# haan6/fm-for-online-recommendation

Measured on NVIDIA B200. Metric: train samples/sec (fwd+bwd+update), higher is better.
Workload: dtype f32

## Files before the change

fm_for_online_recommendation_b200/csrc/fm_backward.cu:

```cuda
#include "fmb_common.cuh"
#include <cstdlib>
#include <cstring>
#include <cuda.h>

namespace {

struct BwdParams {
    const int32_t* skeys;
    const int32_t* perm;
    int64_t N;
    const float* xv;
    float* table;
    int F, k, rowp, kp4;
    int cu;
    int ql_log;
    unsigned long long fmagic;
    int fshift;
    const float* S;
    const float* gs;
    int use_fm2;
    const float* gvec;
    float lr;
    int mode;
    int s_pitch;
    int gs_stride;
    int32_t key_limit;
    float* G;
    int64_t Npad;
    long long* dbg;
    float astep;
    union {
        fmb::FtrlState ftrl;
        fmb::AdagradState ada;
    };
    int min_run1;
    float* inbox[8];
    int shard_G, shard_me;
    int64_t shard_N;
    const int4* run_list;
    const uint32_t* run_segc;
    int run_nseg, run_cap;
    int pdl;
};

template <bool ADA>
__device__ __forceinline__ float row_update(const BwdParams& p, float old, float g, int32_t key, int c) {
    if (ADA) {
        float* sp = p.ada.sums + (size_t)key * p.rowp + c;
        float sv = *sp;
        const float o = fmb::adagrad_update(old, g, sv, p.lr, p.ada.eps);
        *sp = sv;
        return o;
    }
    return fmb::apply_update_a(old, g, p.lr, p.astep, p.mode);
}

template <bool ADA>
__global__ void __launch_bounds__(256) fm_bwd_entry_kernel(BwdParams p) {
    const int q = threadIdx.x & ((1 << p.ql_log) - 1);
    const int64_t i = (int64_t)blockIdx.x * (256 >> p.ql_log) + (threadIdx.x >> p.ql_log);
    if (i >= p.N || q >= p.cu) return;
    const int32_t key = __ldg(p.skeys + i);
    if (key >= p.key_limit) return;
    const int32_t kprev = i > 0 ? __ldg(p.skeys + i - 1) : -1;
    const int32_t knext = i + 1 < p.N ? __ldg(p.skeys + i + 1) : -1;
    const int32_t e = __ldg(p.perm + i);
    const int b = (int)(((unsigned long long)(unsigned)e * p.fmagic) >> p.fshift);
    const float x = p.xv ? __ldg(p.xv + e) : 1.0f;
    const float d = __ldg(p.gs + (size_t)b * p.gs_stride);
    float* rowptr = p.table + (size_t)key * p.rowp + q * 4;
    const float4 v4 = *reinterpret_cast<const float4*>(rowptr);
    float4 s4 = make_float4(0.f, 0.f, 0.f, 0.f), g4 = s4;
    if (q * 4 < p.kp4) {
        s4 = __ldg(reinterpret_cast<const float4*>(p.S + (size_t)b * p.s_pitch + q * 4));
        if (p.gvec) g4 = __ldg(reinterpret_cast<const float4*>(p.gvec + (size_t)b * p.s_pitch + q * 4));
    }
    const float v[4] = {v4.x, v4.y, v4.z, v4.w}, s[4] = {s4.x, s4.y, s4.z, s4.w}, g[4] = {g4.x, g4.y, g4.z, g4.w};
    const bool two = p.use_fm2 && p.gvec;
    float a[4], c[4];
#pragma unroll
    for (int t = 0; t < 4; ++t) {
        const int j = q * 4 + t;
        a[t] = 0.f; c[t] = 0.f;
        if (j < p.k) {
            const float ej = __fmul_rn(v[t], x);
            if (p.use_fm2) a[t] = __fmul_rn(__fsub_rn(__fmul_rn(d, s[t]), __fmul_rn(d, ej)), x);
            if (p.gvec) c[t] = __fmul_rn(__fsub_rn(__fmul_rn(g[t], s[t]), __fmul_rn(g[t], ej)), x);
        } else if (j == p.k) {
            a[t] = __fmul_rn(d, x);
        }
    }
    if (key != kprev && key != knext) {
        float o[4];
#pragma unroll
        for (int t = 0; t < 4; ++t) {
            const int j = q * 4 + t;
            if (j < p.k) {
                const float gr = two ? __fadd_rn(__fadd_rn(0.f, a[t]), __fadd_rn(0.f, c[t]))
                                     : __fadd_rn(0.f, p.gvec ? c[t] : a[t]);
                o[t] = row_update<ADA>(p, v[t], gr, key, j);
            } else if (j == p.k) {
                o[t] = row_update<ADA>(p, v[t], __fadd_rn(0.f, a[t]), key, j);
            } else {
                o[t] = v[t];
            }
        }
        *reinterpret_cast<float4*>(rowptr) = make_float4(o[0], o[1], o[2], o[3]);
    } else {
#pragma unroll
        for (int t = 0; t < 4; ++t) {
            const int j = q * 4 + t;
            if (j > p.k) continue;
            if (two) {
                p.G[(size_t)j * p.Npad + i] = a[t];
                if (j < p.k) p.G[(size_t)(p.k + 1 + j) * p.Npad + i] = c[t];
            } else {
                p.G[(size_t)j * p.Npad + i] = (p.gvec && j < p.k) ? c[t] : a[t];
            }
        }
    }
}

template <int CU, bool ADA>
__global__ void __launch_bounds__(256) fm_bwd_entry1_kernel(BwdParams p) {
    const int64_t i = (int64_t)blockIdx.x * 256 + threadIdx.x;
    if (i >= p.N) return;
    const int32_t key = __ldg(p.skeys + i);
    if (key >= p.key_limit) return;
    const int32_t kprev = i > 0 ? __ldg(p.skeys + i - 1) : -1;
    const int32_t knext = i + 1 < p.N ? __ldg(p.skeys + i + 1) : -1;
    const int32_t e = __ldg(p.perm + i);
    const int b = (int)(((unsigned long long)(unsigned)e * p.fmagic) >> p.fshift);
    const float x = p.xv ? __ldg(p.xv + e) : 1.0f;
    const float d = __ldg(p.gs + (size_t)b * p.gs_stride);
    float* rowptr = p.table + (size_t)key * p.rowp;
    float v[CU * 4], s[CU * 4], g[CU * 4];
#pragma unroll
    for (int q = 0; q < CU; ++q) {
        const float4 v4 = *reinterpret_cast<const float4*>(rowptr + q * 4);
        v[q * 4] = v4.x; v[q * 4 + 1] = v4.y; v[q * 4 + 2] = v4.z; v[q * 4 + 3] = v4.w;
        float4 s4 = make_float4(0.f, 0.f, 0.f, 0.f), g4 = s4;
        if (q * 4 < p.kp4) {
            s4 = __ldg(reinterpret_cast<const float4*>(p.S + (size_t)b * p.s_pitch + q * 4));
            if (p.gvec) g4 = __ldg(reinterpret_cast<const float4*>(p.gvec + (size_t)b * p.s_pitch + q * 4));
        }
        s[q * 4] = s4.x; s[q * 4 + 1] = s4.y; s[q * 4 + 2] = s4.z; s[q * 4 + 3] = s4.w;
        g[q * 4] = g4.x; g[q * 4 + 1] = g4.y; g[q * 4 + 2] = g4.z; g[q * 4 + 3] = g4.w;
    }
    const bool two = p.use_fm2 && p.gvec;
    const bool single = key != kprev && key != knext;
    float o[CU * 4], o2[CU * 4];
#pragma unroll
    for (int j = 0; j < CU * 4; ++j) {
        float a = 0.f, c = 0.f;
        if (j < p.k) {
            const float ej = __fmul_rn(v[j], x);
            if (p.use_fm2) a = __fmul_rn(__fsub_rn(__fmul_rn(d, s[j]), __fmul_rn(d, ej)), x);
            if (p.gvec) c = __fmul_rn(__fsub_rn(__fmul_rn(g[j], s[j]), __fmul_rn(g[j], ej)), x);
        } else if (j == p.k) {
            a = __fmul_rn(d, x);
        }
        if (single) {
            if (j < p.k) {
                const float gr = two ? __fadd_rn(__fadd_rn(0.f, a), __fadd_rn(0.f, c)) : __fadd_rn(0.f, p.gvec ? c : a);
                o[j] = row_update<ADA>(p, v[j], gr, key, j);
            } else if (j == p.k) {
                o[j] = row_update<ADA>(p, v[j], __fadd_rn(0.f, a), key, j);
            } else {
                o[j] = v[j];
            }
        } else {
            o[j] = two ? a : ((p.gvec && j < p.k) ? c : a);
            o2[j] = c;
        }
    }
    if (single) {
#pragma unroll
        for (int q = 0; q < CU; ++q)
            *reinterpret_cast<float4*>(rowptr + q * 4) = make_float4(o[q * 4], o[q * 4 + 1], o[q * 4 + 2], o[q * 4 + 3]);
    } else {
#pragma unroll
        for (int j = 0; j < CU * 4; ++j) {
            if (j > p.k) continue;
            p.G[(size_t)j * p.Npad + i] = o[j];
            if (two && j < p.k) p.G[(size_t)(p.k + 1 + j) * p.Npad + i] = o2[j];
        }
    }
}


__device__ __forceinline__ void mbar_init(uint64_t* bar, int count) {
    asm volatile("mbarrier.init.shared::cta.b64 [%0], %1;\n" ::"r"((unsigned)__cvta_generic_to_shared(bar)), "r"(count));
}
__device__ __forceinline__ void mbar_expect_tx(uint64_t* bar, unsigned bytes) {
    asm volatile("mbarrier.arrive.expect_tx.shared::cta.b64 _, [%0], %1;\n" ::"r"((unsigned)__cvta_generic_to_shared(bar)), "r"(bytes) : "memory");
}
__device__ __forceinline__ bool mbar_wait(uint64_t* bar, unsigned parity) {
    const unsigned a = (unsigned)__cvta_generic_to_shared(bar);
    for (int spin = 0; spin < (1 << 20); ++spin) {
        unsigned ok;
        asm volatile("{\n\t.reg .pred p;\n\tmbarrier.test_wait.parity.shared::cta.b64 p, [%1], %2;\n\tselp.u32 %0, 1, 0, p;\n\t}\n"
                     : "=r"(ok) : "r"(a), "r"(parity) : "memory");
        if (ok) return true;
    }
    return false;
}
__device__ __forceinline__ void tma_g2s_2d(void* smem_dst, const CUtensorMap* tmap, int x, int y, uint64_t* bar) {
    asm volatile(
        "cp.async.bulk.tensor.2d.shared::cluster.global.mbarrier::complete_tx::bytes [%0], [%1, {%2, %3}], [%4];\n" ::"r"(
            (unsigned)__cvta_generic_to_shared(smem_dst)),
        "l"(tmap), "r"(x), "r"(y), "r"((unsigned)__cvta_generic_to_shared(bar))
        : "memory");
}

template <bool LIST, int RING_SE, int RING_NS, bool LONGM, bool ADA>
__device__ __forceinline__ void runs_body(const CUtensorMap& gmap, const BwdParams& p, int warps_per_block, int warp_f, int accs_n,
                                          int ring_comps, unsigned bid, unsigned nblocks, int segb_off) {
    constexpr int RING_SEP = RING_SE + 4;
    extern __shared__ __align__(128) float smem[];
    const int lane = threadIdx.x & 31, wib = threadIdx.x >> 5;
    const int64_t P0 = ((int64_t)bid * warps_per_block + wib) * 32;
    if (!LIST && P0 >= p.N) return;
    const bool two = p.use_fm2 && p.gvec;
    const int kc = p.k + 1;
    const int nv = kc + (two ? p.k : 0);
    const int stage_f = (ring_comps * RING_SEP + 31) & ~31;
    float* ring = smem + (size_t)wib * warp_f;
    uint64_t* bars = reinterpret_cast<uint64_t*>(ring + RING_NS * stage_f);
    float* accs = reinterpret_cast<float*>(bars + RING_NS);

    int32_t k0 = -2, k1 = -2;
    unsigned todo = 0;
    uint32_t lr = 0, ln = 0, lstep = 0;
    uint32_t* seg_base = reinterpret_cast<uint32_t*>(smem + segb_off);
    if (LIST) {
        lr = bid * warps_per_block + wib;
        lstep = nblocks * warps_per_block;
        for (int g = threadIdx.x; g < p.run_nseg; g += blockDim.x) seg_base[g] = __ldg(p.run_segc + (LONGM ? p.run_nseg : 0) + g);
        __syncthreads();
        if (wib == 0) {
            uint32_t carry = 0;
            for (int b0 = 0; b0 < p.run_nseg; b0 += 32) {
                const uint32_t v = b0 + lane < p.run_nseg ? seg_base[b0 + lane] : 0u;
                uint32_t inc = v;
#pragma unroll
                for (int o = 1; o < 32; o <<= 1) { const uint32_t t = __shfl_up_sync(0xffffffffu, inc, o); if (lane >= o) inc += t; }
                if (b0 + lane < p.run_nseg) seg_base[b0 + lane] = carry + inc - v;
                carry += __shfl_sync(0xffffffffu, inc, 31);
            }
            if (lane == 0) seg_base[p.run_nseg] = carry;
        }
        __syncthreads();
        const uint32_t total = seg_base[p.run_nseg];
        ln = total;
        if (wib >= warps_per_block) return;
        if (p.pdl) asm volatile("griddepcontrol.wait;\n" ::: "memory");
    } else {
        const int64_t pos = P0 + lane;
        k0 = pos < p.N ? __ldg(p.skeys + pos) : -2;
        k1 = pos + 32 < p.N ? __ldg(p.skeys + pos + 32) : -2;
        int32_t prev = __shfl_up_sync(0xffffffffu, k0, 1);
        int32_t next = __shfl_down_sync(0xffffffffu, k0, 1);
        const int32_t k1_0 = __shfl_sync(0xffffffffu, k1, 0);
        if (lane == 0) prev = P0 > 0 ? __ldg(p.skeys + P0 - 1) : -1;
        if (lane == 31) next = k1_0;
        todo = __ballot_sync(0xffffffffu, pos < p.N && k0 >= 0 && k0 < p.key_limit && k0 != prev && (k0 == next || p.min_run1));
    }
    bool bars_ready = false;
    unsigned phase = 0;

    while (LIST ? lr < ln : todo != 0) {
        int64_t s;
        int32_t key;
        int n0;
        if (LIST) {
            int lo = 0, hi = p.run_nseg;
            while (hi - lo > 1) { const int mid = (lo + hi) >> 1; if (seg_base[mid] <= lr) lo = mid; else hi = mid; }
            const uint32_t idx = lr - seg_base[lo];
            const int4 e = __ldg(p.run_list + (size_t)lo * p.run_cap + (LONGM ? (uint32_t)p.run_cap - 1u - idx : idx));
            lr += lstep;
            s = e.x; key = e.y; n0 = e.z;
        } else {
            const int bit = __ffs(todo) - 1;
            todo &= todo - 1;
            s = P0 + bit;
            key = __shfl_sync(0xffffffffu, k0, bit);
            const int t = bit + lane;
            const int32_t ka = __shfl_sync(0xffffffffu, k0, t & 31);
            const int32_t kb = __shfl_sync(0xffffffffu, k1, t & 31);
            const unsigned mm = __ballot_sync(0xffffffffu, (t < 32 ? ka : kb) == key);
            n0 = (mm == 0xffffffffu) ? 32 : __ffs(~mm) - 1;
        }
        long long t_start = 0, t_direct = 0, t_ring = 0, c_wait = 0, c_cons = 0, c_issue = 0;
        if (p.dbg) t_start = clock64();
        int run_len = 0;
        int32_t probe = -2;
        const int64_t ring0 = LONGM ? s : s + 32;
        if (LONGM) n0 = 0;
        const bool ringed = LONGM || n0 == 32;
        if (ringed) { const int64_t q = ring0 + 32 * (int64_t)(lane + 1) - 1; probe = q < p.N ? __ldg(p.skeys + q) : -2; }
        if (ringed && !bars_ready) {
            if (lane == 0) {
                for (int st = 0; st < RING_NS; ++st) mbar_init(bars + st, 1);
                asm volatile("fence.mbarrier_init.release.cluster;\n" ::: "memory");
            }
            __syncwarp();
            bars_ready = true;
        }

        for (int v0 = 0; v0 < nv; v0 += 32) {
            const int vl = v0 + lane;
            const bool active = vl < nv;
            const bool isB = vl >= kc;
            const int comp = isB ? vl - kc : vl;
            const float* src = p.G + (size_t)(active ? vl : 0) * p.Npad;
            (void)isB; (void)comp;
            float pold = 0.f;
            if (v0 == 0 && lane < kc && !p.shard_G) pold = p.table[(size_t)key * p.rowp + lane];
            float acc = 0.f;
            {
                const float* sp = src + s;
                float tv[16], tw[16];
#pragma unroll
                for (int u = 0; u < 16; ++u) tv[u] = (active && u < n0) ? __ldg(sp + u) : 0.f;
#pragma unroll
                for (int u = 0; u < 16; ++u) tw[u] = (active && 16 + u < n0) ? __ldg(sp + 16 + u) : 0.f;
#pragma unroll
                for (int u = 0; u < 16; ++u)
                    if (u < n0) acc = __fadd_rn(acc, tv[u]);
#pragma unroll
                for (int u = 0; u < 16; ++u)
                    if (16 + u < n0) acc = __fadd_rn(acc, tw[u]);
            }
            if (p.dbg) t_direct = clock64();
            run_len = n0;
            if (ringed) {
                int64_t c0 = ring0;
                const int mis = (int)(c0 & 3);
                int32_t pr = probe;
                bool ok = true;
                while (ok) {
                    const unsigned pm = __ballot_sync(0xffffffffu, pr == key);
                    const int full = (pm == 0xffffffffu) ? 32 : __ffs(~pm) - 1;
                    int part = 0;
                    if (full < 32) {
                        const int64_t q = c0 + 32 * (int64_t)full + lane;
                        const unsigned m3 = __ballot_sync(0xffffffffu, q < p.N && __ldg(p.skeys + q) == key);
                        part = (m3 == 0xffffffffu) ? 32 : __ffs(~m3) - 1;
                    }
                    const int wlen = 32 * full + part;
                    const int T = (wlen + RING_SE - 1) / RING_SE;
                    auto issue = [&](int tstage) {
                        if (lane == 0) {
                            const int st = tstage & (RING_NS - 1);
                            mbar_expect_tx(bars + st, (unsigned)(ring_comps * RING_SEP * 4));
                            tma_g2s_2d(ring + (size_t)st * stage_f, &gmap, (int)(c0 - mis + RING_SE * (int64_t)tstage), v0, bars + st);
                        }
                    };
                    for (int ts = 0; ts < T && ts < RING_NS; ++ts) issue(ts);
                    int32_t pr_next = -2;
                    if (full == 32) { const int64_t q = c0 + 1024 + 32 * (int64_t)(lane + 1) - 1; pr_next = q < p.N ? __ldg(p.skeys + q) : -2; }
                    for (int ts = 0; ts < T; ++ts) {
                        const int st = ts & (RING_NS - 1);
                        long long w0 = 0;
                        if (p.dbg) w0 = clock64();
                        if (!mbar_wait(bars + st, (phase >> st) & 1u)) { ok = false; break; }
                        phase ^= 1u << st;
                        long long w1 = 0;
                        if (p.dbg) { w1 = clock64(); c_wait += w1 - w0; }
                        const int n = min(RING_SE, wlen - RING_SE * ts);
                        if (active) {
                            const float4* b4 = reinterpret_cast<const float4*>(ring + (size_t)st * stage_f + lane * RING_SEP);
                            if (n == RING_SE) {
                                {
                                    const float4 q = b4[0];
                                    if (mis == 0) acc = __fadd_rn(acc, q.x);
                                    if (mis <= 1) acc = __fadd_rn(acc, q.y);
                                    if (mis <= 2) acc = __fadd_rn(acc, q.z);
                                    acc = __fadd_rn(acc, q.w);
                                }
#pragma unroll
                                for (int c = 0; c < RING_SE / 64; ++c) {
                                    constexpr int last = RING_SE / 64 - 1;
                                    const int nq = c == last ? 15 : 16;
                                    float4 tv[16];
#pragma unroll
                                    for (int u = 0; u < 16; ++u) if (u < nq) tv[u] = b4[1 + 16 * c + u];
#pragma unroll
                                    for (int u = 0; u < 16; ++u)
                                        if (u < nq) {
                                            acc = __fadd_rn(acc, tv[u].x); acc = __fadd_rn(acc, tv[u].y);
                                            acc = __fadd_rn(acc, tv[u].z); acc = __fadd_rn(acc, tv[u].w);
                                        }
                                }
                                {
                                    const float4 q = b4[RING_SE / 4];
                                    if (mis >= 1) acc = __fadd_rn(acc, q.x);
                                    if (mis >= 2) acc = __fadd_rn(acc, q.y);
                                    if (mis >= 3) acc = __fadd_rn(acc, q.z);
                                }
                            } else {
                                const int end = mis + n;
                                int e = 0;
                                if (mis) {
                                    const float4 q = b4[0];
                                    if (mis <= 1 && 1 < end) acc = __fadd_rn(acc, q.y);
                                    if (mis <= 2 && 2 < end) acc = __fadd_rn(acc, q.z);
                                    if (3 < end) acc = __fadd_rn(acc, q.w);
                                    e = 4;
                                }
#pragma unroll 1
                                for (; e + 4 <= end; e += 4) {
                                    const float4 q = b4[e >> 2];
                                    acc = __fadd_rn(acc, q.x); acc = __fadd_rn(acc, q.y);
                                    acc = __fadd_rn(acc, q.z); acc = __fadd_rn(acc, q.w);
                                }
                                if (e < end) {
                                    const float4 q = b4[e >> 2];
                                    acc = __fadd_rn(acc, q.x);
                                    if (e + 1 < end) acc = __fadd_rn(acc, q.y);
                                    if (e + 2 < end) acc = __fadd_rn(acc, q.z);
                                }
                            }
                        }
                        __syncwarp();
                        long long w2 = 0;
                        if (p.dbg) { w2 = clock64(); c_cons += w2 - w1; }
                        if (ts + RING_NS < T) issue(ts + RING_NS);
                        if (p.dbg) c_issue += clock64() - w2;
                    }
                    run_len += wlen;
                    if (full < 32) break;
                    c0 += 1024;
                    pr = pr_next;
                }
            }
            if (p.dbg) t_ring = clock64();
            if (active) accs[vl] = acc;
            if (v0 == 0 && lane < kc) accs[accs_n + lane] = pold;
        }
        __syncwarp();
        for (int c0 = 0; c0 < kc; c0 += 32) {
            const int c = c0 + lane;
            if (c < kc) {
                float gsum = accs[c];
                if (two && c < p.k) gsum = __fadd_rn(gsum, accs[kc + c]);
                if (p.shard_G) {
                    p.inbox[key % p.shard_G][((size_t)p.shard_me * p.shard_N + s) * 16 + c] = gsum;
                    continue;
                }
                float* addr = p.table + (size_t)key * p.rowp + c;
                const float old = c < 32 ? accs[accs_n + c] : *addr;
                if (ADA) {
                    float* sp = p.ada.sums + (size_t)key * p.rowp + c;
                    float sv = *sp;
                    *addr = fmb::adagrad_update(old, gsum, sv, p.lr, p.ada.eps);
                    *sp = sv;
                } else if (p.mode == 2) {
                    float* zp = p.ftrl.zn + (size_t)key * 2 * p.rowp + c;
                    float z = zp[0], n = zp[p.rowp];
                    *addr = fmb::ftrl_update(old, gsum, z, n, p.lr, p.ftrl.beta, p.ftrl.l1, p.ftrl.l2);
                    zp[0] = z; zp[p.rowp] = n;
                } else {
                    *addr = fmb::apply_update_a(old, gsum, p.lr, p.astep, p.mode);
                }
            }
        }
        __syncwarp();
        if (p.dbg && lane == 0 && run_len >= p.dbg[1]) {
            const unsigned long long slot = atomicAdd((unsigned long long*)p.dbg, 1ULL);
            if (slot < 4000) {
                long long* r = p.dbg + 8 + slot * 8;
                unsigned long long gt; asm volatile("mov.u64 %0, %globaltimer;" : "=l"(gt));
                r[0] = run_len; r[1] = (long long)gt - (clock64() - t_start) * 1000 / 1965; r[2] = t_direct - t_start; r[3] = t_ring - t_direct;
                r[4] = clock64() - t_ring; r[5] = c_issue; r[6] = c_wait; r[7] = c_cons;
            }
        }
    }
}

template <bool ADA>
__global__ void __launch_bounds__(256, 2) fm_bwd_runs_kernel(const __grid_constant__ CUtensorMap gmap, BwdParams p, int warps_per_block, int warp_f,
                                                             int accs_n, int ring_comps) {
    runs_body<false, 64, 4, false, ADA>(gmap, p, warps_per_block, warp_f, accs_n, ring_comps, blockIdx.x, gridDim.x, 0);
}

constexpr int LONG_SE = 128, LONG_NS = 4;
template <bool ADA>
__global__ void __launch_bounds__(256, 2) fm_bwd_runs_list_kernel(const __grid_constant__ CUtensorMap gmap_s, const __grid_constant__ CUtensorMap gmap_l,
                                                                  BwdParams p, int wps, int warp_f_s, int wpl, int warp_f_l, int accs_n,
                                                                  int ring_comps, unsigned nlong, int segb_off) {
    if (blockIdx.x < nlong) runs_body<true, LONG_SE, LONG_NS, true, ADA>(gmap_l, p, wpl, warp_f_l, accs_n, ring_comps, blockIdx.x, nlong, segb_off);
    else runs_body<true, 64, 4, false, ADA>(gmap_s, p, wps, warp_f_s, accs_n, ring_comps, blockIdx.x - nlong, gridDim.x - nlong, segb_off);
}

static int ilog2_ceil(int x) { int l = 0; while ((1 << l) < x) ++l; return l; }

}

static int64_t bwd_npad(int64_t N) { return (N + 3) / 4 * 4 + 64; }
FMB_API size_t fmb_bwd_workspace_bytes(int64_t N, int k) {
    const size_t rows = (size_t)((k + 1 + 3) / 4) * 4;
    return 2 * (((size_t)bwd_npad(N) * rows * 4 + 255) / 256 * 256) + 256;
}

static long long* g_runs_dbg = nullptr;
FMB_API void fmb_debug_set_runs_buffer(long long* dev) { g_runs_dbg = dev; }

typedef CUresult (*EncodeTiled)(CUtensorMap*, CUtensorMapDataType, cuuint32_t, void*, const cuuint64_t*, const cuuint64_t*,
                                const cuuint32_t*, const cuuint32_t*, CUtensorMapInterleave, CUtensorMapSwizzle,
                                CUtensorMapL2promotion, CUtensorMapFloatOOBfill);
static EncodeTiled tensor_map_encoder() {
    static EncodeTiled encode = nullptr;
    if (!encode) {
        void* fn = nullptr;
        cudaDriverEntryPointQueryResult qres;
        if (cudaGetDriverEntryPoint("cuTensorMapEncodeTiled", &fn, cudaEnableDefault, &qres) == cudaSuccess && fn) encode = (EncodeTiled)fn;
    }
    return encode;
}

static int ring_warp_floats(int ring_comps, int accs_n, int SE, int NS, int* stage_f_out) {
    const int stage_f = fmb_round_up(ring_comps * (SE + 4), 32);
    if (stage_f_out) *stage_f_out = stage_f;
    return fmb_round_up(NS * stage_f + 2 * NS + accs_n + 32, 32);
}
static int ring_tensor_map(CUtensorMap* gmap, const BwdParams& p, int nv, int ring_comps, int SE) {
    EncodeTiled encode = tensor_map_encoder();
    if (!encode) { fmb_set_error("fmb_fm_backward_update: cuTensorMapEncodeTiled not available from the driver"); return FMB_ERR_CUDA; }
    const cuuint64_t gdim[2] = {(cuuint64_t)p.Npad, (cuuint64_t)nv};
    const cuuint64_t gstride[1] = {(cuuint64_t)p.Npad * 4};
    const cuuint32_t box[2] = {(cuuint32_t)(SE + 4), (cuuint32_t)ring_comps};
    const cuuint32_t estr[2] = {1, 1};
    const CUresult cr = encode(gmap, CU_TENSOR_MAP_DATA_TYPE_FLOAT32, 2, p.G, gdim, gstride, box, estr,
                               CU_TENSOR_MAP_INTERLEAVE_NONE, CU_TENSOR_MAP_SWIZZLE_NONE,
                               CU_TENSOR_MAP_L2_PROMOTION_NONE, CU_TENSOR_MAP_FLOAT_OOB_FILL_NONE);
    if (cr != CUDA_SUCCESS) { fmb_set_error("fmb_fm_backward_update: cuTensorMapEncodeTiled failed (%d)", (int)cr); return FMB_ERR_CUDA; }
    return FMB_OK;
}

template <bool ADA>
static int launch_runs_t(BwdParams& p, bool two, cudaStream_t stream) {
    const int k = p.k;
    const int64_t N = p.N;
    const int nv = k + 1 + (two ? k : 0);
    const int accs_n = (nv + 3) / 4 * 4;
    const int ring_comps = nv < 32 ? nv : 32;
    const int warp_f = ring_warp_floats(ring_comps, accs_n, 64, 4, nullptr);
    int wpb = 8;
    while (wpb > 1 && (size_t)wpb * warp_f * 4 > 56 * 1024) wpb >>= 1;
    const size_t sm = (size_t)wpb * warp_f * 4;
    FMB_CHECK_ARG(sm <= 200 * 1024, "fmb_fm_backward_update: k too large for the run ring");
    const int64_t nwarps = (N + 31) / 32;
    const unsigned grid = (unsigned)((nwarps + wpb - 1) / wpb);
    static bool attr = false;
    if (!attr) {
        cudaFuncSetAttribute(fm_bwd_runs_kernel<ADA>, cudaFuncAttributeMaxDynamicSharedMemorySize, 200 * 1024);
        cudaFuncSetAttribute(fm_bwd_runs_list_kernel<ADA>, cudaFuncAttributeMaxDynamicSharedMemorySize, 200 * 1024);
        attr = true;
    }
    CUtensorMap gmap;
    int rc = ring_tensor_map(&gmap, p, nv, ring_comps, 64);
    if (rc) return rc;
    if (!p.run_list) {
        fm_bwd_runs_kernel<ADA><<<grid, 32 * wpb, sm, stream>>>(gmap, p, wpb, warp_f, accs_n, ring_comps);
        FMB_CHECK_LAUNCH("fm_bwd_runs_kernel");
        return FMB_OK;
    }
    CUtensorMap gmap_l;
    rc = ring_tensor_map(&gmap_l, p, nv, ring_comps, LONG_SE);
    if (rc) return rc;
    const int warp_f_l = ring_warp_floats(ring_comps, accs_n, LONG_SE, LONG_NS, nullptr);
    int wpl = (int)(sm / ((size_t)warp_f_l * 4));
    size_t smd = sm;
    if (wpl < 1) { wpl = 1; smd = (size_t)warp_f_l * 4; }
    if (wpl > wpb) wpl = wpb;
    FMB_CHECK_ARG(smd <= 200 * 1024, "fmb_fm_backward_update: k too large for the long-run ring");
    const size_t segb = (size_t)(p.run_nseg + 1 + 31) / 32 * 128;
    static int sms = 0;
    if (!sms) { int dev = 0; cudaGetDevice(&dev); cudaDeviceGetAttribute(&sms, cudaDevAttrMultiProcessorCount, dev); if (sms <= 0) sms = 148; }
    int per_sm = (int)((size_t)224 * 1024 / (smd + segb + 1024));
    if (per_sm < 1) per_sm = 1;
    if (per_sm * wpb > 32) per_sm = 32 / wpb;
    const unsigned nlong = (unsigned)sms;
    static int short_per_sm = -1;
    if (short_per_sm < 0) { const char* e = getenv("FMB_RUNS_SHORT_PER_SM"); short_per_sm = e ? atoi(e) : 0; }
    unsigned nshort = (unsigned)(sms * (short_per_sm > 0 ? short_per_sm : (per_sm > 1 ? per_sm - 1 : 1)));
    if (nshort > grid) nshort = grid;
    if (p.pdl) {
        cudaLaunchConfig_t cfg;
        memset(&cfg, 0, sizeof(cfg));
        cfg.gridDim = dim3(nlong + nshort); cfg.blockDim = dim3(32 * wpb); cfg.dynamicSmemBytes = smd + segb; cfg.stream = stream;
        cudaLaunchAttribute at[1];
        at[0].id = cudaLaunchAttributeProgrammaticStreamSerialization;
        at[0].val.programmaticStreamSerializationAllowed = 1;
        cfg.attrs = at; cfg.numAttrs = 1;
        const cudaError_t le = cudaLaunchKernelEx(&cfg, fm_bwd_runs_list_kernel<ADA>, gmap, gmap_l, p, wpb, warp_f, wpl, warp_f_l, accs_n,
                                                  ring_comps, nlong, (int)(smd / 4));
        if (le != cudaSuccess) { fmb_set_error("fm_bwd_runs_list_kernel (programmatic launch): %s", cudaGetErrorString(le)); return FMB_ERR_CUDA; }
    } else {
        fm_bwd_runs_list_kernel<ADA><<<nlong + nshort, 32 * wpb, smd + segb, stream>>>(gmap, gmap_l, p, wpb, warp_f, wpl, warp_f_l, accs_n,
                                                                                 ring_comps, nlong, (int)(smd / 4));
    }
    FMB_CHECK_LAUNCH("fm_bwd_runs_list_kernel");
    return FMB_OK;
}
static int launch_runs(BwdParams& p, bool two, cudaStream_t stream) {
    return p.mode == 3 ? launch_runs_t<true>(p, two, stream) : launch_runs_t<false>(p, two, stream);
}

struct fmb_runlist_t { int32_t* entries; uint32_t* seg_count; int nseg, seg_cap; };
struct fmb_adagrad_t { float* sums; float* bias_sum; float* mlp_sums; float eps; };
FMB_API int fmb_fm_backward_update_rl_ex(const int32_t* sorted_keys, const int32_t* perm, int64_t N, int64_t n_entries,
                                         const float* xv, float* table, int F, int k, const float* S, int s_pitch,
                                         const float* gs, int gs_stride, int use_fm2, const float* gvec,
                                         int32_t key_limit, float lr, int mode, const fmb_adagrad_t* ada,
                                         const fmb_runlist_t* rl, void* ws, size_t ws_bytes, cudaStream_t stream) {
    FMB_CHECK_ARG(!rl || (rl->entries && rl->seg_count && rl->nseg >= 1 && rl->nseg <= 2048 && rl->seg_cap >= 1),
                  "fmb_fm_backward_update: bad run list");
    FMB_CHECK_ARG(sorted_keys && perm && table && S && gs && ws, "fmb_fm_backward_update: null pointer");
    FMB_CHECK_ARG(N > 0 && F > 0 && F < 512 && k > 0 && k <= 124, "fmb_fm_backward_update: bad shape N=%lld F=%d k=%d (need F < 512, k <= 124)",
                  (long long)N, F, k);
    FMB_CHECK_ARG(mode == 0 || mode == 1 || (mode == 3 && ada && ada->sums),
                  "fmb_fm_backward_update: unknown update mode %d (mode 3 needs the Adagrad state)", mode);
    FMB_CHECK_ARG(use_fm2 || gvec, "fmb_fm_backward_update: neither gradient path enabled");
    FMB_CHECK_ARG(n_entries > 0 && n_entries < ((int64_t)1 << 31), "fmb_fm_backward_update: n_entries out of range");
    if (ws_bytes < fmb_bwd_workspace_bytes(N, k)) { fmb_set_error("fmb_fm_backward_update: workspace too small"); return FMB_ERR_WS; }
    BwdParams p;
    memset(&p, 0, sizeof(p));
    p.skeys = sorted_keys; p.perm = perm; p.N = N; p.xv = xv; p.table = table;
    p.F = F; p.k = k; p.rowp = fmb_round_up(k + 1, 16); p.kp4 = fmb_round_up(k, 4);
    p.cu = (k + 1 + 3) / 4; p.ql_log = ilog2_ceil(p.cu);
    {
        int bn = 0, bf = 0;
        while (((int64_t)1 << bn) < n_entries) ++bn;
        while ((1 << bf) <= F) ++bf;
        p.fshift = bn + bf;
        p.fmagic = ((1ULL << p.fshift) + (unsigned long long)F - 1) / (unsigned long long)F;
    }
    p.S = S; p.gs = gs; p.use_fm2 = use_fm2; p.gvec = gvec; p.lr = lr; p.mode = mode;
    p.s_pitch = s_pitch; p.gs_stride = gs_stride; p.key_limit = key_limit;
    p.astep = -(lr / 0.1f);
    if (mode == 3) { p.ada.sums = ada->sums; p.ada.bias_sum = ada->bias_sum; p.ada.eps = ada->eps; }
    p.dbg = g_runs_dbg;
    p.Npad = bwd_npad(N);
    p.G = (float*)ws;
    const bool two = use_fm2 && gvec;
    const unsigned grid1 = (unsigned)((N + 255) / 256);
    if (mode == 3) {
        switch (p.cu) {
            case 1: fm_bwd_entry1_kernel<1, true><<<grid1, 256, 0, stream>>>(p); break;
            case 2: fm_bwd_entry1_kernel<2, true><<<grid1, 256, 0, stream>>>(p); break;
            case 3: fm_bwd_entry1_kernel<3, true><<<grid1, 256, 0, stream>>>(p); break;
            case 4: fm_bwd_entry1_kernel<4, true><<<grid1, 256, 0, stream>>>(p); break;
            default: {
                const int epb = 256 >> p.ql_log;
                fm_bwd_entry_kernel<true><<<(unsigned)((N + epb - 1) / epb), 256, 0, stream>>>(p);
            }
        }
    } else {
        switch (p.cu) {
            case 1: fm_bwd_entry1_kernel<1, false><<<grid1, 256, 0, stream>>>(p); break;
            case 2: fm_bwd_entry1_kernel<2, false><<<grid1, 256, 0, stream>>>(p); break;
            case 3: fm_bwd_entry1_kernel<3, false><<<grid1, 256, 0, stream>>>(p); break;
            case 4: fm_bwd_entry1_kernel<4, false><<<grid1, 256, 0, stream>>>(p); break;
            default: {
                const int epb = 256 >> p.ql_log;
                fm_bwd_entry_kernel<false><<<(unsigned)((N + epb - 1) / epb), 256, 0, stream>>>(p);
            }
        }
    }
    FMB_CHECK_LAUNCH("fm_bwd_entry_kernel");
    if (rl) { p.run_list = reinterpret_cast<const int4*>(rl->entries); p.run_segc = rl->seg_count; p.run_nseg = rl->nseg; p.run_cap = rl->seg_cap; }
    return launch_runs(p, two, stream);
}

FMB_API int fmb_fm_backward_update_rl(const int32_t* sorted_keys, const int32_t* perm, int64_t N, int64_t n_entries,
                                      const float* xv, float* table, int F, int k, const float* S, int s_pitch,
                                      const float* gs, int gs_stride, int use_fm2, const float* gvec,
                                      int32_t key_limit, float lr, int mode, const fmb_runlist_t* rl, void* ws, size_t ws_bytes,
                                      cudaStream_t stream) {
    return fmb_fm_backward_update_rl_ex(sorted_keys, perm, N, n_entries, xv, table, F, k, S, s_pitch, gs, gs_stride, use_fm2,
                                        gvec, key_limit, lr, mode, nullptr, rl, ws, ws_bytes, stream);
}

FMB_API int fmb_fm_backward_update_ex(const int32_t* sorted_keys, const int32_t* perm, int64_t N, int64_t n_entries,
                                      const float* xv, float* table, int F, int k, const float* S, int s_pitch,
                                      const float* gs, int gs_stride, int use_fm2, const float* gvec,
                                      int32_t key_limit, float lr, int mode, void* ws, size_t ws_bytes,
                                      cudaStream_t stream) {
    return fmb_fm_backward_update_rl(sorted_keys, perm, N, n_entries, xv, table, F, k, S, s_pitch, gs, gs_stride, use_fm2, gvec,
                                     key_limit, lr, mode, nullptr, ws, ws_bytes, stream);
}

struct fmb_ftrl_t { float* zn; float* bias_zn; float beta, l1, l2; };


static thread_local int g_runs_pdl = 0;
FMB_API void fmb_runs_list_next_is_dependent(int on) { g_runs_pdl = on; }

FMB_API int fmb_fm_backward_runs_list(const int32_t* sorted_keys, int64_t N, float* table, int F, int k, float lr,
                                      int mode, const fmb_ftrl_t* ftrl, const fmb_runlist_t* rl,
                                      void* ws, size_t ws_bytes, cudaStream_t stream) {
    FMB_CHECK_ARG(sorted_keys && table && ws, "fmb_fm_backward_runs: null pointer");
    FMB_CHECK_ARG(!rl || (rl->entries && rl->seg_count && rl->nseg >= 1 && rl->nseg <= 2048 && rl->seg_cap >= 1),
                  "fmb_fm_backward_runs: bad run list");
    FMB_CHECK_ARG(N > 0 && F > 0 && F < 512 && k > 0 && k <= 124, "fmb_fm_backward_runs: bad shape N=%lld F=%d k=%d (need F < 512, k <= 124)",
                  (long long)N, F, k);
    FMB_CHECK_ARG(mode == 0 || mode == 1 || (mode == 2 && ftrl && ftrl->zn) ||
                  (mode == 3 && ftrl && reinterpret_cast<const fmb_adagrad_t*>(ftrl)->sums),
                  "fmb_fm_backward_runs: unknown update mode %d", mode);
    if (ws_bytes < fmb_bwd_workspace_bytes(N, k)) { fmb_set_error("fmb_fm_backward_runs: workspace too small"); return FMB_ERR_WS; }
    BwdParams p;
    memset(&p, 0, sizeof(p));
    p.skeys = sorted_keys; p.N = N; p.table = table;
    p.F = F; p.k = k; p.rowp = fmb_round_up(k + 1, 16); p.kp4 = fmb_round_up(k, 4);
    p.use_fm2 = 1; p.gvec = nullptr; p.lr = lr; p.mode = mode; p.key_limit = 0x7fffffff;
    p.astep = -(lr / 0.1f);
    p.dbg = nullptr;
    p.Npad = bwd_npad(N);
    p.G = (float*)ws;
    if (mode == 2) { p.ftrl.zn = ftrl->zn; p.ftrl.bias_zn = ftrl->bias_zn; p.ftrl.beta = ftrl->beta; p.ftrl.l1 = ftrl->l1; p.ftrl.l2 = ftrl->l2; }
    if (mode == 3) {
        const fmb_adagrad_t* a = reinterpret_cast<const fmb_adagrad_t*>(ftrl);
        p.ada.sums = a->sums; p.ada.bias_sum = a->bias_sum; p.ada.eps = a->eps;
    }
    if (rl) { p.run_list = reinterpret_cast<const int4*>(rl->entries); p.run_segc = rl->seg_count; p.run_nseg = rl->nseg; p.run_cap = rl->seg_cap; }
    p.pdl = rl ? g_runs_pdl : 0;
    g_runs_pdl = 0;
    p.dbg = g_runs_dbg;
    return launch_runs(p, false, stream);
}

FMB_API int fmb_fm_backward_runs_ex(const int32_t* sorted_keys, int64_t N, float* table, int F, int k, float lr,
                                    int mode, const fmb_ftrl_t* ftrl, void* ws, size_t ws_bytes, cudaStream_t stream) {
    return fmb_fm_backward_runs_list(sorted_keys, N, table, F, k, lr, mode, ftrl, nullptr, ws, ws_bytes, stream);
}

FMB_API int fmb_fm_backward_runs(const int32_t* sorted_keys, int64_t N, float* table, int F, int k, float lr,
                                 int mode, void* ws, size_t ws_bytes, cudaStream_t stream) {
    return fmb_fm_backward_runs_ex(sorted_keys, N, table, F, k, lr, mode, nullptr, ws, ws_bytes, stream);
}

FMB_API int fmb_fm_backward_runs_all(const int32_t* sorted_keys, int64_t N, float* table, int F, int k, float lr,
                                     int mode, void* ws, size_t ws_bytes, cudaStream_t stream) {
    FMB_CHECK_ARG(sorted_keys && table && ws, "fmb_fm_backward_runs_all: null pointer");
    FMB_CHECK_ARG(N > 0 && F > 0 && F < 512 && k > 0 && k <= 124, "fmb_fm_backward_runs_all: bad arguments");
    FMB_CHECK_ARG(mode == 0 || mode == 1, "fmb_fm_backward_runs_all: unknown update mode %d", mode);
    if (ws_bytes < fmb_bwd_workspace_bytes(N, k)) { fmb_set_error("fmb_fm_backward_runs_all: workspace too small"); return FMB_ERR_WS; }
    BwdParams p;
    memset(&p, 0, sizeof(p));
    p.skeys = sorted_keys; p.N = N; p.table = table;
    p.F = F; p.k = k; p.rowp = fmb_round_up(k + 1, 16); p.kp4 = fmb_round_up(k, 4);
    p.use_fm2 = 1; p.lr = lr; p.mode = mode; p.key_limit = 0x7fffffff; p.astep = -(lr / 0.1f);
    p.Npad = bwd_npad(N); p.G = (float*)ws; p.min_run1 = 1;
    return launch_runs(p, false, stream);
}

FMB_API int fmb_shard2_runs(const int32_t* sorted_keys, int64_t N, int F, int k, void* ws, size_t ws_bytes,
                            void* const* inbox, int G, int me, cudaStream_t stream) {
    FMB_CHECK_ARG(sorted_keys && ws && inbox, "fmb_shard2_runs: null pointer");
    FMB_CHECK_ARG(N > 0 && F > 0 && F < 512 && k > 0 && k <= 15 && G >= 1 && G <= 8 && me >= 0 && me < G, "fmb_shard2_runs: bad arguments");
    if (ws_bytes < fmb_bwd_workspace_bytes(N, k)) { fmb_set_error("fmb_shard2_runs: workspace too small"); return FMB_ERR_WS; }
    BwdParams p;
    memset(&p, 0, sizeof(p));
    p.skeys = sorted_keys; p.N = N; p.table = nullptr;
    p.F = F; p.k = k; p.rowp = fmb_round_up(k + 1, 16); p.kp4 = fmb_round_up(k, 4);
    p.use_fm2 = 1; p.key_limit = 0x7fffffff;
    p.Npad = bwd_npad(N);
    p.G = (float*)ws;
    for (int o = 0; o < G; ++o) p.inbox[o] = (float*)inbox[o];
    p.shard_G = G; p.shard_me = me; p.shard_N = N;
    return launch_runs(p, false, stream);
}

FMB_API int fmb_fm_backward_update(const int32_t* sorted_keys, const int32_t* perm, int64_t N, const float* xv,
                                   float* table, int F, int k, const float* S, const float* gs, int use_fm2,
                                   const float* gvec, float lr, int mode, void* ws, size_t ws_bytes,
                                   cudaStream_t stream) {
    return fmb_fm_backward_update_ex(sorted_keys, perm, N, N, xv, table, F, k, S, fmb_round_up(k, 4), gs, 1, use_fm2,
                                     gvec, 0x7fffffff, lr, mode, ws, ws_bytes, stream);
}
```

fm_for_online_recommendation_b200/csrc/fm_step.cu:

```cuda
#include "fmb_common.cuh"
#include <cstdlib>

extern "C" size_t fmb_bwd_workspace_bytes(int64_t, int);

namespace {

__device__ __forceinline__ void cp_async16(void* smem, const void* gmem) {
    unsigned s = (unsigned)__cvta_generic_to_shared(smem);
    asm volatile("cp.async.cg.shared.global [%0], [%1], 16;\n" ::"r"(s), "l"(gmem));
}
__device__ __forceinline__ void cp_async_wait_all() {
    asm volatile("cp.async.commit_group;\n" ::);
    asm volatile("cp.async.wait_group 0;\n" ::: "memory");
}

struct StepParams {
    float* table;
    const float* bias;
    int B, F, k, rowp, kp4, SB;
    int cu;
    int ql_log;
    int jl_log;
    uint32_t mF, mcu;
    int loss_kind, mode;
    float lr, astep;
    float* delta;
    float* lossv;
    float* G;
    int64_t Npad;
    union {
        fmb::FtrlState ftrl;
        fmb::AdagradState ada;
    };
    long long* tdbg;
    int dbg;
};

template <int CU, bool XV, int MODE>
__global__ void __launch_bounds__(256, MODE == 2 ? 4 : 8) fm_step_fused_kernel(const int32_t* __restrict__ ids, const float* __restrict__ xv,
                                                            const float* __restrict__ y, const uint32_t* __restrict__ posflag,
                                                            StepParams p) {
    extern __shared__ __align__(16) float smem[];
    const int F = p.F, k = p.k, SB = p.SB;
    const int cu = CU ? CU : p.cu;
    const int rp = cu * 4;
    float* rows_s = smem;
    float* S_s = rows_s + (size_t)SB * F * rp;
    float* x_s = S_s + SB * rp;
    float* bi_s = x_s + (XV ? SB * F : 0);
    float* d_s = bi_s + SB * k;
    int32_t* ids_s = reinterpret_cast<int32_t*>(d_s + SB);
    uint32_t* pos_s = reinterpret_cast<uint32_t*>(ids_s + SB * F);
    uint16_t* single_s = reinterpret_cast<uint16_t*>(pos_s + SB * F);
    uint16_t* multi_s = single_s + SB * F;
    __shared__ int n_single, n_multi;
    if (threadIdx.x == 0) { n_single = 0; n_multi = 0; }
    __syncthreads();
    const int b0 = blockIdx.x * SB;
    const int nv = min(SB, p.B - b0);
    asm volatile("griddepcontrol.launch_dependents;\n" ::);
#define FMB_TS(i) do { if (p.tdbg && threadIdx.x == 0) { unsigned long long t_; asm volatile("mov.u64 %0, %globaltimer;" : "=l"(t_)); p.tdbg[(size_t)blockIdx.x * 8 + (i)] = (long long)t_; } } while (0)
    FMB_TS(0);

    for (int e0 = (threadIdx.x & ~31); e0 < nv * F; e0 += blockDim.x) {
        const int e = e0 + (threadIdx.x & 31);
        const bool valid = e < nv * F;
        uint32_t pf = 0;
        if (valid) {
            ids_s[e] = __ldg(ids + (size_t)b0 * F + e);
            if (XV) x_s[e] = __ldg(xv + (size_t)b0 * F + e);
            pf = __ldg(posflag + (size_t)b0 * F + e);
            pos_s[e] = pf;
        }
        const unsigned ms = __ballot_sync(0xffffffffu, valid && !(pf >> 31));
        const unsigned mm = __ballot_sync(0xffffffffu, valid && (pf >> 31));
        int bs = 0, bm = 0;
        if ((threadIdx.x & 31) == 0) { bs = atomicAdd(&n_single, __popc(ms)); bm = atomicAdd(&n_multi, __popc(mm)); }
        bs = __shfl_sync(0xffffffffu, bs, 0);
        bm = __shfl_sync(0xffffffffu, bm, 0);
        const unsigned lt = (1u << (threadIdx.x & 31)) - 1u;
        if (valid) {
            if (pf >> 31) multi_s[bm + __popc(mm & lt)] = (uint16_t)e;
            else single_s[bs + __popc(ms & lt)] = (uint16_t)e;
        }
    }
    __syncthreads();
    FMB_TS(1);
    {
        const int q = threadIdx.x & ((1 << p.ql_log) - 1);
        const int estep = blockDim.x >> p.ql_log;
        if (q < cu)
            for (int ef = threadIdx.x >> p.ql_log; ef < nv * F; ef += estep)
                cp_async16(rows_s + (size_t)ef * rp + q * 4, p.table + (size_t)ids_s[ef] * p.rowp + q * 4);
    }
    cp_async_wait_all();
    __syncthreads();
    FMB_TS(2);

    {
        const int j = threadIdx.x & ((1 << p.jl_log) - 1);
        const int sstep = blockDim.x >> p.jl_log;
        if (j < p.kp4)
            for (int s = threadIdx.x >> p.jl_log; s < nv; s += sstep) {
                float Sj = 0.f;
                if (j < k) {
                    float Qj = 0.f;
                    const float* r = rows_s + (size_t)s * F * rp + j;
                    const float* xs = x_s + s * F;
#pragma unroll 8
                    for (int f = 0; f < F; ++f) {
                        const float e = XV ? __fmul_rn(r[(size_t)f * rp], xs[f]) : r[(size_t)f * rp];
                        Sj = __fadd_rn(Sj, e);
                        Qj = __fadd_rn(Qj, __fmul_rn(e, e));
                    }
                    bi_s[s * k + j] = __fmul_rn(__fsub_rn(__fmul_rn(Sj, Sj), Qj), 0.5f);
                }
                S_s[s * rp + j] = Sj;
            }
    }
    __syncthreads();
    FMB_TS(3);

    {
        const int s = threadIdx.x >> 3, l8 = threadIdx.x & 7;
        const int nv8 = (nv + 3) & ~3;
        if (s < nv8) {
            const unsigned mask = 0xffffffffu;
            const int sc = min(s, nv - 1);
            const float* r = rows_s + (size_t)sc * F * rp + k;
            const float* xs = x_s + sc * F;
            const float sf = fmb::aten_row_sum_lanes8(
                [&](int f) { return XV ? __fmul_rn(r[(size_t)f * rp], xs[f]) : r[(size_t)f * rp]; }, F, l8, mask);
            const float* bs = bi_s + sc * k;
            const float sb = fmb::aten_row_sum_lanes8([&](int j) { return bs[j]; }, k, l8, mask);
            if (l8 == 0 && s < nv) {
                const int b = b0 + s;
                const float z = __fadd_rn(__fadd_rn(sf, sb), __ldg(p.bias));
                float lv, d;
                fmb::bce_logits_value_grad(p.loss_kind, z, y[b], b, p.B, lv, d);
                p.lossv[b] = lv;
                p.delta[b] = d;
                d_s[s] = d;
            }
        }
    }
    __syncthreads();
    FMB_TS(4);

    const int ns = n_single, nm = n_multi;
    for (int it = threadIdx.x; it < ((p.dbg & 1) ? 0 : ns * cu); it += blockDim.x) {
        const int li = fmb_div_by_magic((unsigned)it, p.mcu), q = it - li * cu;
        const int ef = single_s[li];
        const int s = fmb_div_by_magic((unsigned)ef, p.mF);
        const float x = XV ? x_s[ef] : 1.0f, d = d_s[s];
        const float4 S4 = *reinterpret_cast<const float4*>(S_s + s * rp + q * 4);
        const float4 v4 = *reinterpret_cast<const float4*>(rows_s + (size_t)ef * rp + q * 4);
        const float Sq[4] = {S4.x, S4.y, S4.z, S4.w};
        const float v[4] = {v4.x, v4.y, v4.z, v4.w};
        if (MODE != 2) {
            if (d == 0.0f) continue;
            if (MODE == 0 && !XV && fabsf(d) < 1e-30f && fabsf(p.astep) <= 10.0f) {
                bool same = true;
#pragma unroll
                for (int t = 0; t < 4; ++t) {
                    const int j = q * 4 + t;
                    const float av = fabsf(v[t]);
                    if (j <= k) same = same && av > 1e-9f && av < 1e4f;
                    if (j < k) same = same && fabsf(Sq[t]) < 1e4f;
                }
                if (same) continue;
            }
        }
        if (MODE == 3) {
            float* srow = p.ada.sums + (size_t)ids_s[ef] * p.rowp + q * 4;
            const float4 s4 = *reinterpret_cast<const float4*>(srow);
            float sv[4] = {s4.x, s4.y, s4.z, s4.w}, o[4];
#pragma unroll
            for (int t = 0; t < 4; ++t) {
                const int j = q * 4 + t;
                o[t] = v[t];
                if (j <= k) {
                    float a;
                    if (j < k) {
                        const float ej = XV ? __fmul_rn(v[t], x) : v[t];
                        a = __fsub_rn(__fmul_rn(d, Sq[t]), __fmul_rn(d, ej));
                        if (XV) a = __fmul_rn(a, x);
                    } else {
                        a = XV ? __fmul_rn(d, x) : d;
                    }
                    o[t] = fmb::adagrad_update(v[t], __fadd_rn(0.f, a), sv[t], p.lr, p.ada.eps);
                }
            }
            *reinterpret_cast<float4*>(p.table + (size_t)ids_s[ef] * p.rowp + q * 4) = make_float4(o[0], o[1], o[2], o[3]);
            *reinterpret_cast<float4*>(srow) = make_float4(sv[0], sv[1], sv[2], sv[3]);
            continue;
        }
        float o[4];
        bool moved = false;
        float zz[4] = {0.f, 0.f, 0.f, 0.f}, nn[4] = {0.f, 0.f, 0.f, 0.f};
        float* zrow = nullptr;
        if (MODE == 2) {
            zrow = p.ftrl.zn + (size_t)ids_s[ef] * 2 * p.rowp + q * 4;
            const float4 z4 = *reinterpret_cast<const float4*>(zrow), n4 = *reinterpret_cast<const float4*>(zrow + p.rowp);
            zz[0] = z4.x; zz[1] = z4.y; zz[2] = z4.z; zz[3] = z4.w;
            nn[0] = n4.x; nn[1] = n4.y; nn[2] = n4.z; nn[3] = n4.w;
        }
        float g[4];
#pragma unroll
        for (int t = 0; t < 4; ++t) {
            const int j = q * 4 + t;
            float a = 0.f;
            if (j < k) {
                const float ej = XV ? __fmul_rn(v[t], x) : v[t];
                a = __fsub_rn(__fmul_rn(d, Sq[t]), __fmul_rn(d, ej));
                if (XV) a = __fmul_rn(a, x);
            } else if (j == k) {
                a = XV ? __fmul_rn(d, x) : d;
            }
            g[t] = __fadd_rn(0.f, a);
            o[t] = v[t];
        }
        if (MODE == 2) {
#pragma unroll
            for (int t = 0; t < 4; ++t)
                if (q * 4 + t <= k) {
                    o[t] = fmb::ftrl_update(v[t], g[t], zz[t], nn[t], p.lr, p.ftrl.beta, p.ftrl.l1, p.ftrl.l2);
                    moved = true;
                }
        } else if (MODE == 1) {
#pragma unroll
            for (int t = 0; t < 4; ++t)
                if (q * 4 + t <= k) { o[t] = __fmaf_rn(g[t], -p.lr, v[t]); moved |= __float_as_int(o[t]) != __float_as_int(v[t]); }
        } else {
            unsigned need = 0;
#pragma unroll
            for (int t = 0; t < 4; ++t) {
                float w;
                const bool ok = fmb::adam1_window(v[t], g[t], p.astep, w);
                if (q * 4 + t <= k) { if (ok) o[t] = w; else need |= 1u << t; }
            }
            if (need) {
#pragma unroll
                for (int t = 0; t < 4; ++t)
                    if ((need >> t) & 1u) o[t] = fmb::adam1_rest(v[t], g[t], p.astep, fmb::adam1_in_domain(g[t], p.astep));
            }
#pragma unroll
            for (int t = 0; t < 4; ++t) moved |= __float_as_int(o[t]) != __float_as_int(v[t]);
        }
        if (moved) *reinterpret_cast<float4*>(p.table + (size_t)ids_s[ef] * p.rowp + q * 4) = make_float4(o[0], o[1], o[2], o[3]);
        if (MODE == 2) {
            *reinterpret_cast<float4*>(zrow) = make_float4(zz[0], zz[1], zz[2], zz[3]);
            *reinterpret_cast<float4*>(zrow + p.rowp) = make_float4(nn[0], nn[1], nn[2], nn[3]);
        }
    }
    FMB_TS(5);
    for (int it = threadIdx.x; it < ((p.dbg & 2) ? 0 : nm * cu); it += blockDim.x) {
        const int li = fmb_div_by_magic((unsigned)it, p.mcu), q = it - li * cu;
        const int ef = multi_s[li];
        const int s = fmb_div_by_magic((unsigned)ef, p.mF);
        const float x = XV ? x_s[ef] : 1.0f, d = d_s[s];
        const float4 S4 = *reinterpret_cast<const float4*>(S_s + s * rp + q * 4);
        const float4 v4 = *reinterpret_cast<const float4*>(rows_s + (size_t)ef * rp + q * 4);
        const float Sq[4] = {S4.x, S4.y, S4.z, S4.w};
        const float v[4] = {v4.x, v4.y, v4.z, v4.w};
        float* g = p.G + (size_t)(q * 4) * p.Npad + (pos_s[ef] & 0x7fffffffu);
#pragma unroll
        for (int t = 0; t < 4; ++t) {
            const int j = q * 4 + t;
            if (j < k) {
                const float ej = XV ? __fmul_rn(v[t], x) : v[t];
                float a = __fsub_rn(__fmul_rn(d, Sq[t]), __fmul_rn(d, ej));
                if (XV) a = __fmul_rn(a, x);
                g[(size_t)t * p.Npad] = a;
            } else if (j == k) {
                g[(size_t)t * p.Npad] = XV ? __fmul_rn(d, x) : d;
            }
        }
    }
    FMB_TS(6);
}

__global__ void __launch_bounds__(256) pos_flags_kernel(const int32_t* __restrict__ skeys, const int32_t* __restrict__ perm,
                                                        int64_t N, uint32_t* __restrict__ posflag, int4* __restrict__ run_list,
                                                        uint32_t* __restrict__ run_count, int cap) {
    const int64_t i = (int64_t)blockIdx.x * 256 + threadIdx.x;
    int32_t key = -1;
    bool start = false;
    if (i < N) {
        key = __ldg(skeys + i);
        const int32_t kprev = i > 0 ? __ldg(skeys + i - 1) : -1;
        const int32_t knext = i + 1 < N ? __ldg(skeys + i + 1) : -1;
        const bool multi = key == kprev || key == knext;
        start = multi && key != kprev;
        posflag[__ldg(perm + i)] = (uint32_t)i | (multi ? 0x80000000u : 0u);
    }
    if (!run_list) return;
    const unsigned m = __ballot_sync(0xffffffffu, start);
    if (!m) return;
    const bool lng = start && i + 127 < N && __ldg(skeys + i + 127) == key;
    const unsigned ml = __ballot_sync(0xffffffffu, lng), ms = m & ~ml;
    const int lane = threadIdx.x & 31;
    uint32_t base = 0, basel = 0;
    if (ms) { const int leader = __ffs(ms) - 1; if (lane == leader) base = atomicAdd(run_count, (uint32_t)__popc(ms)); base = __shfl_sync(0xffffffffu, base, leader); }
    if (ml) { const int leader = __ffs(ml) - 1; if (lane == leader) basel = atomicAdd(run_count + 1, (uint32_t)__popc(ml)); basel = __shfl_sync(0xffffffffu, basel, leader); }
    if (start) {
        int n0 = 1;
        bool more = true;
        for (int c = 0; c < 4 && more; ++c) {
            int32_t kk[8];
#pragma unroll
            for (int u = 0; u < 8; ++u) { const int64_t q = i + 1 + c * 8 + u; kk[u] = q < N ? __ldg(skeys + q) : -1; }
#pragma unroll
            for (int u = 0; u < 8; ++u) {
                if (more && c * 8 + u < 31 && kk[u] == key) ++n0; else more = false;
            }
        }
        const uint32_t lt = (1u << lane) - 1u;
        const int4 e4 = make_int4((int)i, key, n0, lng ? 1 : 0);
        if (lng) run_list[(size_t)cap - 1 - (basel + __popc(ml & lt))] = e4;
        else run_list[base + __popc(ms & lt)] = e4;
    }
}

static int ilog2_ceil(int x) { int l = 0; while ((1 << l) < x) ++l; return l; }

}

static int g_step_dbg = 0;
static long long* g_step_tdbg = nullptr;
FMB_API void fmb_debug_set_step_timestamps(long long* dev) { g_step_tdbg = dev; }
FMB_API void fmb_debug_set_step_flags(int f) { g_step_dbg = f; }

typedef void (*fused_fn_t)(const int32_t*, const float*, const float*, const uint32_t*, StepParams);
static fused_fn_t fused_fn(int cu, bool xv, int mode) {
#define FMB_FUSED_ROW(C, X) {fm_step_fused_kernel<C, X, 0>, fm_step_fused_kernel<C, X, 1>, fm_step_fused_kernel<C, X, 2>, \
                             fm_step_fused_kernel<C, X, 3>}
    static const fused_fn_t tab[2][2][4] = {{FMB_FUSED_ROW(0, false), FMB_FUSED_ROW(0, true)},
                                            {FMB_FUSED_ROW(3, false), FMB_FUSED_ROW(3, true)}};
#undef FMB_FUSED_ROW
    return tab[cu == 3][xv][mode];
}
FMB_API int fmb_is_fused_kernel_fn(const void* fn) {
    for (int c = 0; c < 2; ++c)
        for (int x = 0; x < 2; ++x)
            for (int m = 0; m < 4; ++m)
                if (fn == (const void*)fused_fn(c ? 3 : 0, x != 0, m)) return 1;
    return 0;
}
FMB_API const void* fmb_pos_flags_kernel_fn(void) { return (const void*)pos_flags_kernel; }

struct fmb_runlist_t { int32_t* entries; uint32_t* seg_count; int nseg, seg_cap; };
FMB_API int fmb_pos_flags_ex(const int32_t* sorted_keys, const int32_t* perm, int64_t N, uint32_t* posflag,
                             const fmb_runlist_t* rl, cudaStream_t stream) {
    FMB_CHECK_ARG(sorted_keys && perm && posflag && N > 0 && N < ((int64_t)1 << 31), "fmb_pos_flags: bad arguments");
    FMB_CHECK_ARG(!rl || (rl->entries && rl->seg_count && rl->nseg == 1 && rl->seg_cap >= N / 2),
                  "fmb_pos_flags: the run list must be one segment of at least N/2 entries");
    int32_t* run_list = rl ? rl->entries : nullptr;
    uint32_t* run_count = rl ? rl->seg_count : nullptr;
    pos_flags_kernel<<<(unsigned)((N + 255) / 256), 256, 0, stream>>>(sorted_keys, perm, N, posflag,
                                                                      reinterpret_cast<int4*>(run_list), run_count, rl ? rl->seg_cap : 0);
    FMB_CHECK_LAUNCH("pos_flags_kernel");
    return FMB_OK;
}
FMB_API int fmb_pos_flags(const int32_t* sorted_keys, const int32_t* perm, int64_t N, uint32_t* posflag,
                          cudaStream_t stream) {
    return fmb_pos_flags_ex(sorted_keys, perm, N, posflag, nullptr, stream);
}

struct fmb_ftrl_t { float* zn; float* bias_zn; float beta, l1, l2; };
struct fmb_adagrad_t { float* sums; float* bias_sum; float* mlp_sums; float eps; };

FMB_API int fmb_fm_step_fused_ex(const int32_t* ids, const float* xv, const float* y, float* table, const float* bias,
                                 const uint32_t* posflag, int B, int F, int k, int loss_kind, float lr, int mode,
                                 const fmb_ftrl_t* ftrl, float* delta, float* lossv, void* ws, size_t ws_bytes,
                                 cudaStream_t stream) {
    FMB_CHECK_ARG(ids && y && table && bias && posflag && delta && lossv && ws, "fmb_fm_step_fused: null pointer");
    FMB_CHECK_ARG(B > 0 && F > 0 && F < 512 && k > 0 && k <= 124, "fmb_fm_step_fused: bad shape B=%d F=%d k=%d", B, F, k);
    FMB_CHECK_ARG(loss_kind == 0 || loss_kind == 1, "fmb_fm_step_fused: unknown loss kind %d", loss_kind);
    FMB_CHECK_ARG(mode == 0 || mode == 1 || (mode == 2 && ftrl && ftrl->zn) ||
                  (mode == 3 && ftrl && reinterpret_cast<const fmb_adagrad_t*>(ftrl)->sums),
                  "fmb_fm_step_fused: unknown update mode %d (mode 2 needs the FTRL state, mode 3 the Adagrad state)", mode);
    const int64_t N = (int64_t)B * F;
    if (ws_bytes < fmb_bwd_workspace_bytes(N, k)) { fmb_set_error("fmb_fm_step_fused: workspace too small"); return FMB_ERR_WS; }
    StepParams p;
    p.table = table; p.bias = bias;
    p.B = B; p.F = F; p.k = k; p.rowp = fmb_round_up(k + 1, 16); p.kp4 = fmb_round_up(k, 4);
    p.cu = (k + 1 + 3) / 4; p.ql_log = ilog2_ceil(p.cu); p.jl_log = ilog2_ceil(p.kp4);
    p.mF = fmb_div_magic((unsigned)F); p.mcu = fmb_div_magic((unsigned)p.cu);
    p.loss_kind = loss_kind; p.mode = mode; p.lr = lr; p.astep = -(lr / 0.1f);
    p.delta = delta; p.lossv = lossv;
    p.G = (float*)ws; p.Npad = (N + 3) / 4 * 4 + 64;
    p.dbg = g_step_dbg;
    p.ftrl.zn = nullptr; p.ftrl.bias_zn = nullptr; p.ftrl.beta = p.ftrl.l1 = p.ftrl.l2 = 0.f;
    if (mode == 2) { p.ftrl.zn = ftrl->zn; p.ftrl.bias_zn = ftrl->bias_zn; p.ftrl.beta = ftrl->beta; p.ftrl.l1 = ftrl->l1; p.ftrl.l2 = ftrl->l2; }
    if (mode == 3) { const fmb_adagrad_t* a = reinterpret_cast<const fmb_adagrad_t*>(ftrl); p.ada.sums = a->sums; p.ada.bias_sum = a->bias_sum; p.ada.eps = a->eps; }
    p.tdbg = g_step_tdbg;
    int SB = 256 >> p.jl_log;
    if (SB < 4) SB = 4;
    if (SB > 32) SB = 32;
    auto bytes = [&](int sb) {
        return sizeof(float) * ((size_t)sb * F * p.cu * 4 + (size_t)4 * sb * F + (size_t)sb * k + (size_t)sb * p.cu * 4 + sb);
    };
    while (SB > 1 && bytes(SB) > 48 * 1024) SB >>= 1;
    while (SB > 8) SB >>= 1;
    {
        static int cap = -1;
        if (cap < 0) { const char* e = getenv("FMB_STEP_SB"); cap = e ? atoi(e) : 0; }
        if (cap > 0 && SB > cap) SB = cap;
    }
    FMB_CHECK_ARG(bytes(SB) <= 200 * 1024, "fmb_fm_step_fused: F*k too large for one sample tile (F=%d k=%d: %zu bytes > 200 KB)",
                  F, k, bytes(SB));
    p.SB = SB;
    const fused_fn_t fn = fused_fn(p.cu, xv != nullptr, mode);
    if (bytes(SB) > 48 * 1024) cudaFuncSetAttribute(fn, cudaFuncAttributeMaxDynamicSharedMemorySize, 200 * 1024);
    fn<<<(B + SB - 1) / SB, 256, bytes(SB), stream>>>(ids, xv, y, posflag, p);
    FMB_CHECK_LAUNCH("fm_step_fused_kernel");
    return FMB_OK;
}

FMB_API int fmb_fm_step_fused(const int32_t* ids, const float* xv, const float* y, float* table, const float* bias,
                              const uint32_t* posflag, int B, int F, int k, int loss_kind, float lr, int mode,
                              float* delta, float* lossv, void* ws, size_t ws_bytes, cudaStream_t stream) {
    return fmb_fm_step_fused_ex(ids, xv, y, table, bias, posflag, B, F, k, loss_kind, lr, mode, nullptr, delta, lossv, ws,
                                ws_bytes, stream);
}
```

fm_for_online_recommendation_b200/csrc/session.cu:

```cuda
#include "fmb_common.cuh"
#include <cstdlib>
#include <cstring>
#include <cstddef>
#include <new>

extern "C" {
int fmb_fm_forward(const int32_t*, const float*, const float*, const float*, int, int, int, float*, float*, float*,
                   float*, float*, const float*, int, float*, float*, cudaStream_t);
size_t fmb_sort_workspace_bytes(int64_t);
int fmb_sort_segment(const int32_t*, int64_t, int, void*, size_t, int32_t*, int32_t*, int32_t*, int32_t*,
                     cudaStream_t);
size_t fmb_bwd_workspace_bytes(int64_t, int);
int fmb_sort_fields_max_batch(void);
struct fmb_runlist_t { int32_t* entries; uint32_t* seg_count; int nseg, seg_cap; };
void fmb_runlist_shape(int, int, int*, int*);
int fmb_sort_fields_ex(const int32_t*, int, int, const int32_t*, int32_t*, int32_t*, uint32_t*, const fmb_runlist_t*, int, cudaStream_t);
int fmb_pos_flags_ex(const int32_t*, const int32_t*, int64_t, uint32_t*, const fmb_runlist_t*, cudaStream_t);
int fmb_fm_backward_update(const int32_t*, const int32_t*, int64_t, const float*, float*, int, int, const float*,
                           const float*, int, const float*, float, int, void*, size_t, cudaStream_t);
int fmb_finish_step(const float*, const float*, int, float*, float, int, float*, cudaStream_t);
struct fmb_ftrl_t { float* zn; float* bias_zn; float beta, l1, l2; };
struct fmb_adagrad_t { float* sums; float* bias_sum; float* mlp_sums; float eps; };
int fmb_fm_backward_runs_list(const int32_t*, int64_t, float*, int, int, float, int, const fmb_ftrl_t*, const fmb_runlist_t*,
                              void*, size_t, cudaStream_t);
int fmb_finish_step_ex(const float*, const float*, int, float*, float, int, const fmb_ftrl_t*, float*, cudaStream_t);
int fmb_fm_step_fused_ex(const int32_t*, const float*, const float*, float*, const float*, const uint32_t*, int, int, int,
                         int, float, int, const fmb_ftrl_t*, float*, float*, void*, size_t, cudaStream_t);
int fmb_fm_backward_runs_ex(const int32_t*, int64_t, float*, int, int, float, int, const fmb_ftrl_t*, void*, size_t,
                            cudaStream_t);
int fmb_pos_flags(const int32_t*, const int32_t*, int64_t, uint32_t*, cudaStream_t);
int fmb_fm_step_fused(const int32_t*, const float*, const float*, float*, const float*, const uint32_t*, int, int, int,
                      int, float, int, float*, float*, void*, size_t, cudaStream_t);
int fmb_fm_backward_runs(const int32_t*, int64_t, float*, int, int, float, int, void*, size_t, cudaStream_t);
int fmb_is_fused_kernel_fn(const void*);
void fmb_runs_list_next_is_dependent(int);
const void* fmb_finish_kernel_fn(void);
int fmb_sort_fields_kernel_fns(const void**, int*, int*);
}

#define FMB_GRAPH_CACHE 32
struct StepVariant {
    int B, key_bits, loss_kind, mode, has_xv, pre, has_next, cur;
    const void *table, *bias;
    float lr;
    cudaGraph_t graph;
    cudaGraphExec_t exec;
    cudaGraphNode_t n_fused, n_finish, n_sort_cur[2], n_sort_next[2];
    int np_sort_cur[2], np_sort_next[2];
    int nlaunch;
    const void *cur_ids, *cur_xv, *cur_y, *cur_sort_ids, *cur_next_ids, *cur_loss;
};

struct fmb_session {
    int F, k, rowp, kp4;
    int64_t maxB;
    int32_t* d_ids;
    float* d_xv;
    float* d_y;
    float* d_S;
    float* d_z;
    float* d_delta;
    float* d_lossv;
    float* d_loss;
    int32_t* d_skeys;
    int32_t* d_perm;
    int32_t* d_skeys_buf[2];
    int32_t* d_perm_buf[2];
    uint32_t* d_posflag_buf[2];
    int32_t* d_runlist_buf[2];
    uint32_t* d_runcount_buf[2];
    int rl_nseg, rl_cap;
    void* d_sort_ws2;
    const int32_t* presort_ids;
    int presort_B, presort_buf, last_buf;
    int presort_ext;
    int presort_stale;
    cudaEvent_t ev_presort, ev_buf_free[2];
    int buf_used[2];
    void* d_sort_ws;
    size_t sort_ws_bytes;
    void* d_bwd_ws;
    size_t bwd_ws_bytes;
    int32_t* d_field_off;
    int32_t* h_ids;
    float* h_xv;
    float* h_y;
    float* h_loss;
    int32_t* d_ids2; float* d_xv2; float* d_y2; float* d_loss2;
    int32_t* h_ids2; float* h_xv2; float* h_y2;
    int32_t* d_idsx[2]; float* d_xvx[2]; float* d_yx[2];
    int32_t* h_idsx[2]; float* h_xvx[2]; float* h_yx[2];
    cudaStream_t st_copy;
    cudaEvent_t ev_h2d[4], ev_done[4];
    int slot_used[4];
    int64_t launches;
    cudaStream_t st0, st1, st2, st3, st4;
    cudaEvent_t ev_sp_fork, ev_sp_join, ev_join4;
    int64_t steps_done;
    cudaEvent_t ev_fork, ev_fwd, ev_sort, ev_join;
    int use_graph, use_prio;
    int host_path;
    int use_pdl;
    int sort_after;
    int sparse_ok;
    int ngraphs, next_evict;
    StepVariant gvar[FMB_GRAPH_CACHE];
    cudaEvent_t ev_join2;
    struct { const int32_t* ids; int B, key_bits, buf, nl; cudaGraphExec_t exec; cudaGraph_t graph; } psg[8];
    int npsg, presort_warm;
    fmb_ftrl_t ftrl;
    int ftrl_set;
    fmb_adagrad_t ada;
    int ada_set;
};

#define CU(call)                                                                              \
    do {                                                                                      \
        cudaError_t e__ = (call);                                                             \
        if (e__ != cudaSuccess) { fmb_set_error("%s: %s", #call, cudaGetErrorString(e__)); return FMB_ERR_CUDA; } \
    } while (0)

FMB_API void fmb_session_destroy(fmb_session* s) {
    if (!s) return;
    cudaFree(s->d_ids); cudaFree(s->d_xv); cudaFree(s->d_y); cudaFree(s->d_S); cudaFree(s->d_z);
    cudaFree(s->d_delta); cudaFree(s->d_lossv); cudaFree(s->d_loss);
    for (int i = 0; i < 2; ++i) { cudaFree(s->d_skeys_buf[i]); cudaFree(s->d_perm_buf[i]); cudaFree(s->d_posflag_buf[i]); cudaFree(s->d_runlist_buf[i]); cudaFree(s->d_runcount_buf[i]); if (s->ev_buf_free[i]) cudaEventDestroy(s->ev_buf_free[i]); }
    cudaFree(s->d_sort_ws2);
    if (s->ev_join2) cudaEventDestroy(s->ev_join2);
    for (int i = 0; i < s->npsg; ++i) if (s->psg[i].exec) { cudaGraphExecDestroy(s->psg[i].exec); cudaGraphDestroy(s->psg[i].graph); }
    if (s->ev_sp_fork) cudaEventDestroy(s->ev_sp_fork);
    if (s->ev_sp_join) cudaEventDestroy(s->ev_sp_join);
    if (s->st3) cudaStreamDestroy(s->st3);
    if (s->st4) cudaStreamDestroy(s->st4);
    if (s->ev_join4) cudaEventDestroy(s->ev_join4);
    if (s->ev_presort) cudaEventDestroy(s->ev_presort);
    cudaFree(s->d_sort_ws); cudaFree(s->d_bwd_ws); cudaFree(s->d_field_off);
    cudaFreeHost(s->h_ids); cudaFreeHost(s->h_xv); cudaFreeHost(s->h_y); cudaFreeHost(s->h_loss);
    cudaFree(s->d_ids2); cudaFree(s->d_xv2); cudaFree(s->d_y2); cudaFree(s->d_loss2);
    cudaFreeHost(s->h_ids2); cudaFreeHost(s->h_xv2); cudaFreeHost(s->h_y2);
    if (s->st_copy) cudaStreamDestroy(s->st_copy);
    for (int i = 0; i < 4; ++i) { if (s->ev_h2d[i]) cudaEventDestroy(s->ev_h2d[i]); if (s->ev_done[i]) cudaEventDestroy(s->ev_done[i]); }
    for (int i = 0; i < 2; ++i) {
        cudaFree(s->d_idsx[i]); cudaFree(s->d_xvx[i]); cudaFree(s->d_yx[i]);
        cudaFreeHost(s->h_idsx[i]); cudaFreeHost(s->h_xvx[i]); cudaFreeHost(s->h_yx[i]);
    }
    for (int i = 0; i < s->ngraphs; ++i) { cudaGraphExecDestroy(s->gvar[i].exec); cudaGraphDestroy(s->gvar[i].graph); }
    if (s->st0) cudaStreamDestroy(s->st0);
    if (s->st1) cudaStreamDestroy(s->st1);
    if (s->st2) cudaStreamDestroy(s->st2);
    if (s->ev_fork) cudaEventDestroy(s->ev_fork);
    if (s->ev_fwd) cudaEventDestroy(s->ev_fwd);
    if (s->ev_sort) cudaEventDestroy(s->ev_sort);
    if (s->ev_join) cudaEventDestroy(s->ev_join);
    delete s;
}

FMB_API int fmb_session_create(fmb_session** out, int F, int k, int64_t max_batch, const int32_t* field_off_host) {
    FMB_CHECK_ARG(out && F > 0 && k > 0 && max_batch > 0, "fmb_session_create: bad arguments");
    FMB_CHECK_ARG(max_batch * F < ((int64_t)1 << 31), "fmb_session_create: max_batch*F must fit int32");
    fmb_session* s = new (std::nothrow) fmb_session();
    FMB_CHECK_ARG(s, "fmb_session_create: out of host memory");
    memset(s, 0, sizeof(*s));
    s->F = F; s->k = k; s->rowp = fmb_round_up(k + 1, 16); s->kp4 = fmb_round_up(k, 4); s->maxB = max_batch;
    const int64_t N = max_batch * F;
    fmb_runlist_shape((int)(max_batch < 65536 ? max_batch : 65536), F, &s->rl_nseg, &s->rl_cap);
    if ((int64_t)s->rl_nseg * s->rl_cap < N / 2 + 64) s->rl_cap = (int)((N / 2 + 64 + s->rl_nseg - 1) / s->rl_nseg);
    s->sort_ws_bytes = fmb_sort_workspace_bytes(N);
    s->bwd_ws_bytes = fmb_bwd_workspace_bytes(N, k);
    cudaError_t e = cudaSuccess;
    auto dm = [&](void** p, size_t n) { if (e == cudaSuccess) e = cudaMalloc(p, n); };
    auto hm = [&](void** p, size_t n) { if (e == cudaSuccess) e = cudaMallocHost(p, n); };
    dm((void**)&s->d_ids, N * 4); dm((void**)&s->d_xv, N * 4); dm((void**)&s->d_y, max_batch * 4);
    dm((void**)&s->d_S, max_batch * s->kp4 * 4); dm((void**)&s->d_z, max_batch * 4);
    dm((void**)&s->d_delta, max_batch * 4); dm((void**)&s->d_lossv, max_batch * 4); dm((void**)&s->d_loss, 256);
    for (int i = 0; i < 2; ++i) { dm((void**)&s->d_skeys_buf[i], N * 4); dm((void**)&s->d_perm_buf[i], N * 4); dm((void**)&s->d_posflag_buf[i], N * 4); dm((void**)&s->d_runlist_buf[i], (size_t)s->rl_nseg * s->rl_cap * 16); dm((void**)&s->d_runcount_buf[i], (size_t)s->rl_nseg * 8 + 256); }
    if (!(field_off_host && max_batch <= fmb_sort_fields_max_batch())) dm(&s->d_sort_ws2, s->sort_ws_bytes);
    s->d_skeys = s->d_skeys_buf[0]; s->d_perm = s->d_perm_buf[0];
    dm(&s->d_sort_ws, s->sort_ws_bytes); dm(&s->d_bwd_ws, s->bwd_ws_bytes);
    hm((void**)&s->h_ids, N * 4); hm((void**)&s->h_xv, N * 4); hm((void**)&s->h_y, max_batch * 4);
    hm((void**)&s->h_loss, 256);
    dm((void**)&s->d_ids2, N * 4); dm((void**)&s->d_xv2, N * 4); dm((void**)&s->d_y2, max_batch * 4);
    dm((void**)&s->d_loss2, 256);
    hm((void**)&s->h_ids2, N * 4); hm((void**)&s->h_xv2, N * 4); hm((void**)&s->h_y2, max_batch * 4);
    if (e == cudaSuccess) e = cudaStreamCreateWithFlags(&s->st_copy, cudaStreamNonBlocking);
    for (int i = 0; i < 4; ++i) {
        if (e == cudaSuccess) e = cudaEventCreateWithFlags(&s->ev_h2d[i], cudaEventDisableTiming);
        if (e == cudaSuccess) e = cudaEventCreateWithFlags(&s->ev_done[i], cudaEventDisableTiming);
    }
    if (field_off_host) {
        dm((void**)&s->d_field_off, (size_t)(F + 1) * 4);
        if (e == cudaSuccess) e = cudaMemcpy(s->d_field_off, field_off_host, (size_t)(F + 1) * 4, cudaMemcpyHostToDevice);
    }
    {
        int least = 0, greatest = 0;
        const char* pe = getenv("FMB_PRIO");
        s->use_prio = pe ? atoi(pe) : 1;
        if (s->use_prio && cudaDeviceGetStreamPriorityRange(&least, &greatest) != cudaSuccess) s->use_prio = 0;
        if (!s->use_prio) least = greatest = 0;
        if (s->use_prio == 1) { const int t = least; least = greatest; greatest = t; }
        if (e == cudaSuccess) e = cudaStreamCreateWithPriority(&s->st0, cudaStreamNonBlocking, greatest);
        if (e == cudaSuccess) e = cudaStreamCreateWithPriority(&s->st1, cudaStreamNonBlocking, greatest);
        if (e == cudaSuccess) e = cudaStreamCreateWithPriority(&s->st2, cudaStreamNonBlocking, least);
        if (e == cudaSuccess) e = cudaStreamCreateWithPriority(&s->st3, cudaStreamNonBlocking, least);
        if (e == cudaSuccess) e = cudaStreamCreateWithPriority(&s->st4, cudaStreamNonBlocking, greatest);
        if (e == cudaSuccess) e = cudaEventCreateWithFlags(&s->ev_join4, cudaEventDisableTiming);
        if (e == cudaSuccess) e = cudaEventCreateWithFlags(&s->ev_sp_fork, cudaEventDisableTiming);
        if (e == cudaSuccess) e = cudaEventCreateWithFlags(&s->ev_sp_join, cudaEventDisableTiming);
    }
    if (e == cudaSuccess) e = cudaEventCreateWithFlags(&s->ev_fork, cudaEventDisableTiming);
    if (e == cudaSuccess) e = cudaEventCreateWithFlags(&s->ev_fwd, cudaEventDisableTiming);
    if (e == cudaSuccess) e = cudaEventCreateWithFlags(&s->ev_sort, cudaEventDisableTiming);
    if (e == cudaSuccess) e = cudaEventCreateWithFlags(&s->ev_join, cudaEventDisableTiming);
    if (e == cudaSuccess) e = cudaEventCreateWithFlags(&s->ev_presort, cudaEventDisableTiming);
    if (e == cudaSuccess) e = cudaEventCreateWithFlags(&s->ev_join2, cudaEventDisableTiming);
    for (int i = 0; i < 2; ++i) if (e == cudaSuccess) e = cudaEventCreateWithFlags(&s->ev_buf_free[i], cudaEventDisableTiming);
    {
        const char* ng = getenv("FMB_NO_GRAPH");
        s->use_graph = !(ng && ng[0] == '1');
        const char* sp = getenv("FMB_SPARSE");
        s->sparse_ok = !(sp && sp[0] == '0');
        const char* pd = getenv("FMB_PDL");
        s->use_pdl = !(pd && pd[0] == '0');
        const char* sa = getenv("FMB_SORT_AFTER");
        s->sort_after = sa && sa[0] == '1';
    }
    if (e != cudaSuccess) {
        fmb_set_error("fmb_session_create: %s", cudaGetErrorString(e));
        fmb_session_destroy(s);
        return FMB_ERR_CUDA;
    }
    *out = s;
    return FMB_OK;
}

FMB_API int fmb_session_set_ftrl(fmb_session* s, float* zn_dev, float* bias_zn_dev, float beta, float l1, float l2) {
    FMB_CHECK_ARG(s && zn_dev && bias_zn_dev && l1 >= 0.f && l2 >= 0.f, "fmb_session_set_ftrl: bad arguments");
    s->ftrl.zn = zn_dev; s->ftrl.bias_zn = bias_zn_dev; s->ftrl.beta = beta; s->ftrl.l1 = l1; s->ftrl.l2 = l2;
    s->ftrl_set = 1;
    for (int i = 0; i < s->ngraphs; ++i) { cudaGraphExecDestroy(s->gvar[i].exec); cudaGraphDestroy(s->gvar[i].graph); }
    s->ngraphs = 0; s->next_evict = 0;
    return FMB_OK;
}

FMB_API int fmb_session_set_adagrad(fmb_session* s, float* sums_dev, float* bias_sum_dev, float eps) {
    FMB_CHECK_ARG(s && sums_dev && bias_sum_dev && eps >= 0.f, "fmb_session_set_adagrad: bad arguments");
    s->ada.sums = sums_dev; s->ada.bias_sum = bias_sum_dev; s->ada.mlp_sums = nullptr; s->ada.eps = eps;
    s->ada_set = 1;
    for (int i = 0; i < s->ngraphs; ++i) { cudaGraphExecDestroy(s->gvar[i].exec); cudaGraphDestroy(s->gvar[i].graph); }
    s->ngraphs = 0; s->next_evict = 0;
    return FMB_OK;
}

FMB_API int64_t fmb_session_launches(const fmb_session* s) { return s ? s->launches : 0; }
FMB_API int fmb_session_graph_count(const fmb_session* s) { return s ? s->ngraphs : 0; }

static bool by_field_sort(const fmb_session* s, int B) { return s->d_field_off && B <= fmb_sort_fields_max_batch(); }

static int sort_launch(fmb_session* s, const int32_t* ids, int B, int key_bits, int buf, void* radix_ws,
                       cudaStream_t st, int* nlaunch) {
    const int64_t N = (int64_t)B * s->F;
    int rc;
    fmb_runlist_t rl;
    rl.entries = s->d_runlist_buf[buf]; rl.seg_count = s->d_runcount_buf[buf];
    if (by_field_sort(s, B)) {
        fmb_runlist_shape(B, s->F, &rl.nseg, &rl.seg_cap);
        if (!s->sparse_ok) {
            *nlaunch += 1;
            return fmb_sort_fields_ex(ids, B, s->F, s->d_field_off, s->d_skeys_buf[buf], s->d_perm_buf[buf],
                                      s->d_posflag_buf[buf], &rl, 0, st);
        }
        cudaMemsetAsync(s->d_posflag_buf[buf], 0, (size_t)N * 4, st);
        cudaEventRecord(s->ev_sp_fork, st);
        cudaStreamWaitEvent(s->st3, s->ev_sp_fork, 0);
        rc = fmb_sort_fields_ex(ids, B, s->F, s->d_field_off, s->d_skeys_buf[buf], s->d_perm_buf[buf], s->d_posflag_buf[buf],
                                &rl, 1 | 2, st);
        if (rc) return rc;
        rc = fmb_sort_fields_ex(ids, B, s->F, s->d_field_off, s->d_skeys_buf[buf], s->d_perm_buf[buf], s->d_posflag_buf[buf],
                                &rl, 1 | 4, s->st3);
        cudaEventRecord(s->ev_sp_join, s->st3);
        cudaStreamWaitEvent(st, s->ev_sp_join, 0);
        *nlaunch += 2;
        return rc;
    } else {
        rc = fmb_sort_segment(ids, N, key_bits, radix_ws, s->sort_ws_bytes, s->d_skeys_buf[buf], s->d_perm_buf[buf],
                              nullptr, nullptr, st);
        *nlaunch += 3 * ((key_bits + 7) / 8);
    }
    if (rc) return rc;
    rl.nseg = 1; rl.seg_cap = (int)(N / 2 + 1);
    cudaMemsetAsync(s->d_runcount_buf[buf], 0, 8, st);
    rc = fmb_pos_flags_ex(s->d_skeys_buf[buf], s->d_perm_buf[buf], N, s->d_posflag_buf[buf], &rl, st);
    *nlaunch += 1;
    return rc;
}

static int fm_step_launch(fmb_session* s, const int32_t* ids, const float* xv, const float* y, int B, float* table,
                          float* bias, int key_bits, int loss_kind, float lr, int mode, float* loss_dev,
                          const int32_t* next_ids, cudaStream_t main, cudaStream_t side, cudaStream_t side2, int cur,
                          bool pre, int* nlaunch) {
    const int64_t N = (int64_t)B * s->F;
    int rc;
    *nlaunch = 0;
    cudaEventRecord(s->ev_fork, main);
    cudaStreamWaitEvent(side, s->ev_fork, 0);
    if (next_ids && !s->sort_after) {
        cudaStreamWaitEvent(side2, s->ev_fork, 0);
        rc = sort_launch(s, next_ids, B, key_bits, 1 - cur, s->d_sort_ws2, side2, nlaunch);
        if (rc) return rc;
        cudaEventRecord(s->ev_join2, side2);
    }
    if (!pre) {
        rc = sort_launch(s, ids, B, key_bits, cur, s->d_sort_ws, main, nlaunch);
        if (rc) return rc;
    }
    const fmb_ftrl_t* ft = mode == 3 ? (s->ada_set ? reinterpret_cast<const fmb_ftrl_t*>(&s->ada) : nullptr)
                                     : (s->ftrl_set ? &s->ftrl : nullptr);
    rc = fmb_fm_step_fused_ex(ids, xv, y, table, bias, s->d_posflag_buf[cur], B, s->F, s->k, loss_kind, lr, mode, ft,
                              s->d_delta, s->d_lossv, s->d_bwd_ws, s->bwd_ws_bytes, main);
    if (rc) return rc;
    cudaEventRecord(s->ev_fwd, main);
    cudaStreamWaitEvent(side, s->ev_fwd, 0);
    if (next_ids && s->sort_after) {
        cudaStreamWaitEvent(side2, s->ev_fwd, 0);
        rc = sort_launch(s, next_ids, B, key_bits, 1 - cur, s->d_sort_ws2, side2, nlaunch);
        if (rc) return rc;
        cudaEventRecord(s->ev_join2, side2);
    }
    rc = fmb_finish_step_ex(s->d_delta, s->d_lossv, B, bias, lr, mode, ft, loss_dev ? loss_dev : s->d_loss, side);
    if (rc) return rc;
    cudaEventRecord(s->ev_join, side);
    fmb_runlist_t rl;
    rl.entries = s->d_runlist_buf[cur]; rl.seg_count = s->d_runcount_buf[cur];
    if (by_field_sort(s, B)) fmb_runlist_shape(B, s->F, &rl.nseg, &rl.seg_cap);
    else { rl.nseg = 1; rl.seg_cap = (int)(N / 2 + 1); }
    fmb_runs_list_next_is_dependent(s->use_pdl);
    rc = fmb_fm_backward_runs_list(s->d_skeys_buf[cur], N, table, s->F, s->k, lr, mode, ft, &rl, s->d_bwd_ws, s->bwd_ws_bytes, main);
    if (rc) return rc;
    cudaStreamWaitEvent(main, s->ev_join, 0);
    if (next_ids) cudaStreamWaitEvent(main, s->ev_join2, 0);
    *nlaunch += 3;
    return FMB_OK;
}

static int patch_node(cudaGraphExec_t exec, cudaGraphNode_t node, int nparams, const void* const* repl) {
    cudaKernelNodeParams kp;
    CU(cudaGraphKernelNodeGetParams(node, &kp));
    void* args[16];
    for (int i = 0; i < nparams; ++i) args[i] = repl[i] ? const_cast<void*>(repl[i]) : kp.kernelParams[i];
    kp.kernelParams = args;
    kp.extra = nullptr;
    CU(cudaGraphExecKernelNodeSetParams(exec, node, &kp));
    return FMB_OK;
}

static int capture_variant(fmb_session* s, StepVariant* v, const int32_t* ids, const float* xv, const float* y,
                           float* table, float* bias, const int32_t* next_ids) {
    cudaGraph_t graph = nullptr;
    int nl = 0;
    CU(cudaStreamBeginCapture(s->st0, cudaStreamCaptureModeThreadLocal));
    const int rc = fm_step_launch(s, ids, xv, y, v->B, table, bias, v->key_bits, v->loss_kind, v->lr, v->mode, s->d_loss,
                                  next_ids, s->st0, s->st1, s->st2, v->cur, v->pre != 0, &nl);
    cudaError_t e = cudaStreamEndCapture(s->st0, &graph);
    if (rc) { if (graph) cudaGraphDestroy(graph); return rc; }
    if (e != cudaSuccess) { fmb_set_error("graph capture: %s", cudaGetErrorString(e)); return FMB_ERR_CUDA; }
    cudaGraphNode_t nodes[64];
    size_t nn = 64;
    CU(cudaGraphGetNodes(graph, nodes, &nn));
    const void* sort_fns[8];
    int sort_np[8], sort_ska[8];
    const int nsort = fmb_sort_fields_kernel_fns(sort_fns, sort_np, sort_ska);
    v->n_fused = v->n_finish = nullptr;
    for (int j = 0; j < 2; ++j) v->n_sort_cur[j] = v->n_sort_next[j] = nullptr;
    for (size_t i = 0; i < nn; ++i) {
        cudaGraphNodeType ty;
        CU(cudaGraphNodeGetType(nodes[i], &ty));
        if (ty != cudaGraphNodeTypeKernel) continue;
        cudaKernelNodeParams kp;
        CU(cudaGraphKernelNodeGetParams(nodes[i], &kp));
        if (fmb_is_fused_kernel_fn(kp.func)) { v->n_fused = nodes[i]; continue; }
        if (kp.func == fmb_finish_kernel_fn()) { v->n_finish = nodes[i]; continue; }
        for (int t = 0; t < nsort; ++t)
            if (kp.func == sort_fns[t]) {
                const int32_t* out = *static_cast<int32_t**>(kp.kernelParams[sort_ska[t]]);
                const bool is_cur = out == s->d_skeys_buf[v->cur];
                cudaGraphNode_t* dst = is_cur ? v->n_sort_cur : v->n_sort_next;
                int* dnp = is_cur ? v->np_sort_cur : v->np_sort_next;
                const int j = dst[0] ? 1 : 0;
                dst[j] = nodes[i]; dnp[j] = sort_np[t];
            }
    }
    if (!v->n_fused || !v->n_finish || (!v->pre && !v->n_sort_cur[0]) || (v->has_next && !v->n_sort_next[0])) {
        cudaGraphDestroy(graph);
        fmb_set_error("step graph: kernel nodes not found");
        return FMB_ERR_CUDA;
    }
    cudaGraphExec_t exec = nullptr;
    e = cudaGraphInstantiate(&exec, graph, s->use_prio ? cudaGraphInstantiateFlagUseNodePriority : 0);
    if (e != cudaSuccess) { cudaGraphDestroy(graph); fmb_set_error("graph instantiate: %s", cudaGetErrorString(e)); return FMB_ERR_CUDA; }
    v->graph = graph; v->exec = exec; v->nlaunch = nl;
    return FMB_OK;
}

FMB_API int fmb_session_fm_step_next(fmb_session* s, const int32_t* ids, const float* xv, const float* y, int B,
                                     float* table, float* bias, int key_bits, int loss_kind, float lr, int mode,
                                     const int32_t* next_ids, float* loss_dev, cudaStream_t stream) {
    FMB_CHECK_ARG(s && ids && y && table && bias, "fmb_session_fm_step: null pointer");
    FMB_CHECK_ARG(B > 0 && B <= s->maxB, "fmb_session_fm_step: B=%d exceeds session max_batch", B);
    int nl = 0;
    const bool pre = s->presort_ids == ids && s->presort_B == B && !s->presort_stale;
    s->presort_stale = 0;
    const int cur = pre ? s->presort_buf : 1 - s->last_buf;
    if (pre) {
        if (s->presort_ext) CU(cudaStreamWaitEvent(stream, s->ev_presort, 0));
    } else {
        if (s->buf_used[cur]) CU(cudaStreamWaitEvent(stream, s->ev_buf_free[cur], 0));
        if (s->presort_ids && s->presort_ext) CU(cudaStreamWaitEvent(stream, s->ev_presort, 0));
    }
    s->presort_ids = nullptr;
    if (next_ids && s->buf_used[1 - cur]) CU(cudaStreamWaitEvent(stream, s->ev_buf_free[1 - cur], 0));
    s->last_buf = cur;
    int rc = FMB_OK;
    if (!s->use_graph || s->steps_done == 0 || !by_field_sort(s, B)) {
        rc = fm_step_launch(s, ids, xv, y, B, table, bias, key_bits, loss_kind, lr, mode, loss_dev, next_ids, stream,
                            s->st1, s->st2, cur, pre, &nl);
        if (rc) return rc;
        s->launches += nl;
    } else {
        StepVariant key;
        memset(&key, 0, sizeof(key));
        key.B = B; key.key_bits = key_bits; key.loss_kind = loss_kind; key.mode = mode; key.has_xv = xv != nullptr;
        key.pre = pre; key.has_next = next_ids != nullptr; key.cur = cur; key.table = table; key.bias = bias; key.lr = lr;
        StepVariant* v = nullptr;
        const size_t keylen = offsetof(StepVariant, graph);
        float* want_loss = loss_dev ? loss_dev : s->d_loss;
        int same_key = 0;
        for (int i = 0; i < s->ngraphs; ++i)
            if (memcmp(&s->gvar[i], &key, keylen) == 0) {
                ++same_key;
                if (!v) v = &s->gvar[i];
                if (s->gvar[i].cur_ids == ids && s->gvar[i].cur_y == y && s->gvar[i].cur_loss == want_loss) { v = &s->gvar[i]; same_key = 99; break; }
            }
        if (v && same_key < 4 && s->host_path) v = nullptr;
        if (!v) {
            rc = capture_variant(s, &key, ids, xv, y, table, bias, next_ids);
            if (rc) return rc;
            int slot;
            if (s->ngraphs < FMB_GRAPH_CACHE) slot = s->ngraphs++;
            else {
                slot = s->next_evict; s->next_evict = (s->next_evict + 1) % FMB_GRAPH_CACHE;
                cudaGraphExecDestroy(s->gvar[slot].exec); cudaGraphDestroy(s->gvar[slot].graph);
            }
            s->gvar[slot] = key;
            v = &s->gvar[slot];
        }
        if (v->cur_ids != ids || v->cur_xv != xv || v->cur_y != y) {
            const void* repl[16] = {nullptr};
            repl[0] = &ids; repl[1] = &xv; repl[2] = &y;
            rc = patch_node(v->exec, v->n_fused, 5, repl);
            if (rc) return rc;
            v->cur_ids = ids; v->cur_xv = xv; v->cur_y = y;
        }
        if (!pre && v->cur_sort_ids != ids) {
            const void* repl[16] = {nullptr};
            repl[0] = &ids;
            for (int j = 0; j < 2 && v->n_sort_cur[j]; ++j) {
                rc = patch_node(v->exec, v->n_sort_cur[j], v->np_sort_cur[j], repl);
                if (rc) return rc;
            }
            v->cur_sort_ids = ids;
        }
        if (next_ids && v->cur_next_ids != next_ids) {
            const void* repl[16] = {nullptr};
            repl[0] = &next_ids;
            for (int j = 0; j < 2 && v->n_sort_next[j]; ++j) {
                rc = patch_node(v->exec, v->n_sort_next[j], v->np_sort_next[j], repl);
                if (rc) return rc;
            }
            v->cur_next_ids = next_ids;
        }
        {
            float* lo = loss_dev ? loss_dev : s->d_loss;
            if (v->cur_loss != lo) {
                const void* repl[16] = {nullptr};
                repl[6] = &lo;
                rc = patch_node(v->exec, v->n_finish, 9, repl);
                if (rc) return rc;
                v->cur_loss = lo;
            }
        }
        CU(cudaGraphLaunch(v->exec, stream));
        s->launches += v->nlaunch;
    }
    CU(cudaEventRecord(s->ev_buf_free[cur], stream));
    s->buf_used[cur] = 1;
    if (next_ids) {
        s->presort_ids = next_ids; s->presort_B = B; s->presort_buf = 1 - cur; s->presort_ext = 0;
        CU(cudaEventRecord(s->ev_buf_free[1 - cur], stream));
        s->buf_used[1 - cur] = 1;
    }
    s->steps_done += 1;
    return FMB_OK;
}

FMB_API int fmb_session_fm_step(fmb_session* s, const int32_t* ids, const float* xv, const float* y, int B,
                                float* table, float* bias, int key_bits, int loss_kind, float lr, int mode,
                                float* loss_dev, cudaStream_t stream) {
    return fmb_session_fm_step_next(s, ids, xv, y, B, table, bias, key_bits, loss_kind, lr, mode, nullptr, loss_dev, stream);
}

static int presort_impl(fmb_session* s, const int32_t* ids, int B, int key_bits, cudaEvent_t ready) {
    const int buf = 1 - s->last_buf;
    if (s->buf_used[buf]) CU(cudaStreamWaitEvent(s->st2, s->ev_buf_free[buf], 0));
    if (ready) CU(cudaStreamWaitEvent(s->st2, ready, 0));
    int nl = 0;
    if (s->use_graph && s->presort_warm && by_field_sort(s, B)) {
        int g = -1;
        for (int i = 0; i < s->npsg; ++i)
            if (s->psg[i].ids == ids && s->psg[i].B == B && s->psg[i].key_bits == key_bits && s->psg[i].buf == buf) g = i;
        if (g < 0) {
            cudaGraph_t graph = nullptr;
            CU(cudaStreamBeginCapture(s->st2, cudaStreamCaptureModeThreadLocal));
            const int rc = sort_launch(s, ids, B, key_bits, buf, s->d_sort_ws2 ? s->d_sort_ws2 : s->d_sort_ws, s->st2, &nl);
            const cudaError_t e = cudaStreamEndCapture(s->st2, &graph);
            if (rc) { if (graph) cudaGraphDestroy(graph); return rc; }
            if (e != cudaSuccess) { fmb_set_error("pre-sort graph capture: %s", cudaGetErrorString(e)); return FMB_ERR_CUDA; }
            cudaGraphExec_t exec = nullptr;
            if (cudaGraphInstantiate(&exec, graph, 0) != cudaSuccess) { cudaGraphDestroy(graph); fmb_set_error("pre-sort graph instantiate failed"); return FMB_ERR_CUDA; }
            g = s->npsg < 8 ? s->npsg++ : 0;
            if (s->psg[g].exec) { cudaGraphExecDestroy(s->psg[g].exec); cudaGraphDestroy(s->psg[g].graph); }
            s->psg[g].ids = ids; s->psg[g].B = B; s->psg[g].key_bits = key_bits; s->psg[g].buf = buf; s->psg[g].nl = nl;
            s->psg[g].exec = exec; s->psg[g].graph = graph;
        }
        nl = s->psg[g].nl;
        CU(cudaGraphLaunch(s->psg[g].exec, s->st2));
    } else {
        const int rc = sort_launch(s, ids, B, key_bits, buf, s->d_sort_ws2 ? s->d_sort_ws2 : s->d_sort_ws, s->st2, &nl);
        if (rc) return rc;
        s->presort_warm = 1;
    }
    CU(cudaEventRecord(s->ev_presort, s->st2));
    s->launches += nl;
    s->presort_ids = ids; s->presort_B = B; s->presort_buf = buf; s->presort_ext = 1;
    return FMB_OK;
}

FMB_API int fmb_session_presort(fmb_session* s, const int32_t* ids, int B, int key_bits) {
    FMB_CHECK_ARG(s && ids && B > 0 && B <= s->maxB, "fmb_session_presort: bad arguments");
    return presort_impl(s, ids, B, key_bits, nullptr);
}

FMB_API void fmb_session_presort_invalidate(fmb_session* s) {
    if (!s || !s->presort_ids) return;
    s->presort_stale = 1;
}

static bool host_ptr_is_pinned(const void* p) {
    static thread_local const void* seen[16];
    static thread_local bool pinned[16];
    static thread_local int nseen = 0, nextw = 0;
    for (int i = 0; i < nseen; ++i) if (seen[i] == p) return pinned[i];
    cudaPointerAttributes a;
    bool r = false;
    if (cudaPointerGetAttributes(&a, p) != cudaSuccess) cudaGetLastError();
    else r = a.type == cudaMemoryTypeHost;
    seen[nextw] = p; pinned[nextw] = r; nextw = (nextw + 1) % 16; if (nseen < 16) ++nseen;
    return r;
}
FMB_API int fmb_session_fm_step_host_async(fmb_session* s, int slot, const int32_t* ids_host, const float* xv_host,
                                           const float* y_host, int B, float* table, float* bias, int key_bits,
                                           int loss_kind, float lr, int mode, cudaStream_t stream) {
    FMB_CHECK_ARG(s && ids_host && y_host && table && bias, "fmb_session_fm_step_host_async: null pointer");
    FMB_CHECK_ARG(slot >= 0 && slot < 4, "fmb_session_fm_step_host_async: slot must be 0..3");
    FMB_CHECK_ARG(B > 0 && B <= s->maxB, "fmb_session_fm_step_host_async: B=%d exceeds session max_batch", B);
    const size_t N = (size_t)B * s->F;
    if (slot >= 2 && !s->d_idsx[slot - 2]) {
        const size_t NN = (size_t)s->maxB * s->F;
        const int j = slot - 2;
        cudaError_t e = cudaMalloc((void**)&s->d_idsx[j], NN * 4);
        if (e == cudaSuccess) e = cudaMalloc((void**)&s->d_xvx[j], NN * 4);
        if (e == cudaSuccess) e = cudaMalloc((void**)&s->d_yx[j], (size_t)s->maxB * 4);
        if (e == cudaSuccess) e = cudaMallocHost((void**)&s->h_idsx[j], NN * 4);
        if (e == cudaSuccess) e = cudaMallocHost((void**)&s->h_xvx[j], NN * 4);
        if (e == cudaSuccess) e = cudaMallocHost((void**)&s->h_yx[j], (size_t)s->maxB * 4);
        if (e != cudaSuccess) { fmb_set_error("fmb_session_fm_step_host_async: %s", cudaGetErrorString(e)); return FMB_ERR_CUDA; }
    }
    int32_t* d_ids = slot >= 2 ? s->d_idsx[slot - 2] : (slot ? s->d_ids2 : s->d_ids);
    float* d_xv = slot >= 2 ? s->d_xvx[slot - 2] : (slot ? s->d_xv2 : s->d_xv);
    float* d_y = slot >= 2 ? s->d_yx[slot - 2] : (slot ? s->d_y2 : s->d_y);
    float* d_loss = slot ? s->d_loss2 : s->d_loss;
    int32_t* h_ids = slot >= 2 ? s->h_idsx[slot - 2] : (slot ? s->h_ids2 : s->h_ids);
    float* h_xv = slot >= 2 ? s->h_xvx[slot - 2] : (slot ? s->h_xv2 : s->h_xv);
    float* h_y = slot >= 2 ? s->h_yx[slot - 2] : (slot ? s->h_y2 : s->h_y);
    if (s->slot_used[slot]) CU(cudaEventSynchronize(s->ev_done[slot]));
    const void* src_ids = ids_host;
    const void* src_y = y_host;
    const void* src_xv = xv_host;
    if (!host_ptr_is_pinned(ids_host)) { memcpy(h_ids, ids_host, N * 4); src_ids = h_ids; }
    if (!host_ptr_is_pinned(y_host)) { memcpy(h_y, y_host, (size_t)B * 4); src_y = h_y; }
    if (xv_host && !host_ptr_is_pinned(xv_host)) { memcpy(h_xv, xv_host, N * 4); src_xv = h_xv; }
    CU(cudaMemcpyAsync(d_ids, src_ids, N * 4, cudaMemcpyHostToDevice, s->st_copy));
    CU(cudaMemcpyAsync(d_y, src_y, (size_t)B * 4, cudaMemcpyHostToDevice, s->st_copy));
    if (xv_host) CU(cudaMemcpyAsync(d_xv, src_xv, N * 4, cudaMemcpyHostToDevice, s->st_copy));
    CU(cudaEventRecord(s->ev_h2d[slot], s->st_copy));
    CU(cudaStreamWaitEvent(stream, s->ev_h2d[slot], 0));
    int rc = presort_impl(s, d_ids, B, key_bits, s->ev_h2d[slot]);
    if (rc) return rc;
    (void)d_loss;
    s->host_path = 1;
    rc = fmb_session_fm_step(s, d_ids, xv_host ? d_xv : nullptr, d_y, B, table, bias, key_bits, loss_kind, lr,
                                 mode, s->h_loss + 8 * slot, stream);
    s->host_path = 0;
    if (rc) return rc;
    CU(cudaEventRecord(s->ev_done[slot], stream));
    s->slot_used[slot] = 1;
    return FMB_OK;
}

FMB_API int fmb_session_host_slots(void) { return 4; }

FMB_API int fmb_session_wait_loss(fmb_session* s, int slot, float* loss_host) {
    FMB_CHECK_ARG(s && slot >= 0 && slot < 4 && s->slot_used[slot], "fmb_session_wait_loss: nothing submitted on slot %d", slot);
    CU(cudaEventSynchronize(s->ev_done[slot]));
    if (loss_host) *loss_host = s->h_loss[8 * slot];
    return FMB_OK;
}

FMB_API int fmb_session_fm_step_host(fmb_session* s, const int32_t* ids_host, const float* xv_host,
                                     const float* y_host, int B, float* table, float* bias, int key_bits,
                                     int loss_kind, float lr, int mode, float* loss_host, cudaStream_t stream) {
    FMB_CHECK_ARG(s && ids_host && y_host && table && bias, "fmb_session_fm_step_host: null pointer");
    FMB_CHECK_ARG(B > 0 && B <= s->maxB, "fmb_session_fm_step_host: B=%d exceeds session max_batch", B);
    const size_t N = (size_t)B * s->F;
    memcpy(s->h_ids, ids_host, N * 4);
    memcpy(s->h_y, y_host, (size_t)B * 4);
    CU(cudaMemcpyAsync(s->d_ids, s->h_ids, N * 4, cudaMemcpyHostToDevice, stream));
    CU(cudaMemcpyAsync(s->d_y, s->h_y, (size_t)B * 4, cudaMemcpyHostToDevice, stream));
    if (xv_host) {
        memcpy(s->h_xv, xv_host, N * 4);
        CU(cudaMemcpyAsync(s->d_xv, s->h_xv, N * 4, cudaMemcpyHostToDevice, stream));
    }
    int rc = fmb_session_fm_step(s, s->d_ids, xv_host ? s->d_xv : nullptr, s->d_y, B, table, bias, key_bits,
                                 loss_kind, lr, mode, s->d_loss, stream);
    if (rc) return rc;
    CU(cudaMemcpyAsync(s->h_loss, s->d_loss, 4, cudaMemcpyDeviceToHost, stream));
    CU(cudaStreamSynchronize(stream));
    if (loss_host) *loss_host = s->h_loss[0];
    return FMB_OK;
}
```

Measured before the change: 203.4 million.

## Stream backward run kernel against fused kernel via per-tile epoch flags

The fused step kernel now publishes per-tile completion flags tagged with a per-step epoch. The backward runs-list kernel no longer waits for the whole fused grid through griddepcontrol. Each warp instead polls only the flags of the tiles its run entries need, either with an exact wait or a frontier scan for long runs, before issuing TMA loads. This lets the run updates overlap the tail of the fused kernel, at the cost of spin-polling, extra fences, per-step graph node patching for the epoch, and a timeout error path.

```diff
diff --git a/fm_for_online_recommendation_b200/csrc/fm_backward.cu b/fm_for_online_recommendation_b200/csrc/fm_backward.cu
--- a/fm_for_online_recommendation_b200/csrc/fm_backward.cu
+++ b/fm_for_online_recommendation_b200/csrc/fm_backward.cu
@@ -41,6 +41,9 @@
     const uint32_t* run_segc;
     int run_nseg, run_cap;
     int pdl;
+    const uint32_t* sflags;
+    uint32_t tile_div;
+    int* err;
 };
 
 template <bool ADA>
@@ -213,9 +216,84 @@
         : "memory");
 }
 
+constexpr int WAIT_SPINS = 1 << 22;
+
+__device__ __forceinline__ bool poll_tile(const BwdParams& p, uint32_t t, int lane, uint32_t epoch, int& spins) {
+    bool ok = true;
+    if (lane == 0) {
+        for (;; ++spins) {
+            uint32_t v;
+            asm volatile("ld.relaxed.gpu.global.u32 %0, [%1];\n" : "=r"(v) : "l"(p.sflags + t));
+            if (v == epoch) break;
+            if (spins >= WAIT_SPINS) { ok = false; break; }
+            __nanosleep(256);
+        }
+    }
+    return __shfl_sync(0xffffffffu, ok, 0);
+}
+
+template <int U>
+__device__ bool wait_exact(const BwdParams& p, int64_t a, int64_t b, int lane, uint32_t epoch) {
+    uint32_t t[U];
+#pragma unroll
+    for (int u = 0; u < U; ++u) { const int64_t i = a + lane + 32 * u; t[u] = i < b ? (uint32_t)__ldg(p.perm + i) : ~0u; }
+#pragma unroll
+    for (int u = 0; u < U; ++u) if (t[u] != ~0u) t[u] /= p.tile_div;
+    for (int spins = 0;;) {
+        uint32_t late = 0;
+#pragma unroll
+        for (int u = 0; u < U; ++u)
+            if (t[u] != ~0u) {
+                uint32_t v;
+                asm volatile("ld.relaxed.gpu.global.u32 %0, [%1];\n" : "=r"(v) : "l"(p.sflags + t[u]));
+                if (v == epoch) t[u] = ~0u; else late = max(late, t[u] + 1);
+            }
+        late = __reduce_max_sync(0xffffffffu, late);
+        if (!late) break;
+        if (!poll_tile(p, late - 1, lane, epoch, spins)) return false;
+    }
+    asm volatile("fence.acq_rel.gpu;\n" ::: "memory");
+    return true;
+}
+
+template <int U>
+__device__ __forceinline__ void frontier_load(const BwdParams& p, uint32_t tnext, uint32_t lim, int lane, uint32_t epoch, uint32_t (&f)[U]) {
+#pragma unroll
+    for (int u = 0; u < U; ++u) {
+        const uint32_t t = tnext + lane + 32 * u;
+        f[u] = epoch;
+        if (t <= lim) asm volatile("ld.relaxed.gpu.global.u32 %0, [%1];\n" : "=r"(f[u]) : "l"(p.sflags + t));
+    }
+}
+template <int U>
+__device__ __forceinline__ uint32_t frontier_count(const uint32_t (&f)[U], uint32_t tnext, uint32_t lim, uint32_t epoch) {
+    uint32_t pre = 32 * U;
+#pragma unroll
+    for (int u = U - 1; u >= 0; --u) {
+        const unsigned m = __ballot_sync(0xffffffffu, f[u] != epoch);
+        if (m) pre = 32 * u + __ffs(m) - 1;
+    }
+    return min(pre, lim + 1 - tnext);
+}
+__device__ bool wait_frontier(const BwdParams& p, uint32_t& tnext, uint32_t need, uint32_t lim, int lane, uint32_t epoch) {
+    if (need < tnext) return true;
+    int spins = 0;
+    for (;;) {
+        uint32_t f[16];
+        frontier_load(p, tnext, lim, lane, epoch, f);
+        const uint32_t pre = frontier_count(f, tnext, lim, epoch);
+        tnext += pre;
+        if (pre == 512 && tnext <= lim) continue;
+        if (tnext > need) break;
+        if (!poll_tile(p, tnext, lane, epoch, spins)) return false;
+    }
+    asm volatile("fence.acq_rel.gpu;\n" ::: "memory");
+    return true;
+}
+
 template <bool LIST, int RING_SE, int RING_NS, bool LONGM, bool ADA>
 __device__ __forceinline__ void runs_body(const CUtensorMap& gmap, const BwdParams& p, int warps_per_block, int warp_f, int accs_n,
-                                          int ring_comps, unsigned bid, unsigned nblocks, int segb_off) {
+                                          int ring_comps, unsigned bid, unsigned nblocks, int segb_off, uint32_t epoch) {
     constexpr int RING_SEP = RING_SE + 4;
     extern __shared__ __align__(128) float smem[];
     const int lane = threadIdx.x & 31, wib = threadIdx.x >> 5;
@@ -232,6 +310,10 @@
     int32_t k0 = -2, k1 = -2;
     unsigned todo = 0;
     uint32_t lr = 0, ln = 0, lstep = 0;
+    bool streaming = LIST && p.sflags;
+    auto waited = [&](bool ok) {
+        if (!ok) { if (lane == 0) { *(volatile int*)p.err = 1; __threadfence_system(); } streaming = false; }
+    };
     uint32_t* seg_base = reinterpret_cast<uint32_t*>(smem + segb_off);
     if (LIST) {
         lr = bid * warps_per_block + wib;
@@ -254,7 +336,7 @@
         const uint32_t total = seg_base[p.run_nseg];
         ln = total;
         if (wib >= warps_per_block) return;
-        if (p.pdl) asm volatile("griddepcontrol.wait;\n" ::: "memory");
+        if (p.pdl && !p.sflags) asm volatile("griddepcontrol.wait;\n" ::: "memory");
     } else {
         const int64_t pos = P0 + lane;
         k0 = pos < p.N ? __ldg(p.skeys + pos) : -2;
@@ -317,14 +399,20 @@
             (void)isB; (void)comp;
             float pold = 0.f;
             if (v0 == 0 && lane < kc && !p.shard_G) pold = p.table[(size_t)key * p.rowp + lane];
+            const bool wait_now = streaming && v0 == 0;
+            uint32_t tnext = 0;
+            if (!LONGM && wait_now && n0 > 0) {
+                waited(wait_exact<1>(p, s, s + n0, lane, epoch));
+                __syncwarp();
+            }
             float acc = 0.f;
             {
                 const float* sp = src + s;
                 float tv[16], tw[16];
 #pragma unroll
-                for (int u = 0; u < 16; ++u) tv[u] = (active && u < n0) ? __ldg(sp + u) : 0.f;
-#pragma unroll
-                for (int u = 0; u < 16; ++u) tw[u] = (active && 16 + u < n0) ? __ldg(sp + 16 + u) : 0.f;
+                for (int u = 0; u < 16; ++u) tv[u] = (active && u < n0) ? (LIST ? __ldcg(sp + u) : __ldg(sp + u)) : 0.f;
+#pragma unroll
+                for (int u = 0; u < 16; ++u) tw[u] = (active && 16 + u < n0) ? (LIST ? __ldcg(sp + 16 + u) : __ldg(sp + 16 + u)) : 0.f;
 #pragma unroll
                 for (int u = 0; u < 16; ++u)
                     if (u < n0) acc = __fadd_rn(acc, tv[u]);
@@ -357,11 +445,50 @@
                             tma_g2s_2d(ring + (size_t)st * stage_f, &gmap, (int)(c0 - mis + RING_SE * (int64_t)tstage), v0, bars + st);
                         }
                     };
-                    for (int ts = 0; ts < T && ts < RING_NS; ++ts) issue(ts);
+                    const int64_t wend = c0 + wlen;
+                    const bool front = LONGM && wait_now && streaming;
+                    uint32_t needl = 0, lim = 0;
+                    int issued = 0;
+                    if (front) {
+                        const int64_t q = lane < T ? min(c0 + RING_SE * (int64_t)(lane + 1), wend) - 1 : c0;
+                        needl = (uint32_t)__ldg(p.perm + q) / p.tile_div;
+                        tnext = max(tnext, __shfl_sync(0xffffffffu, needl, 31));
+                        lim = __shfl_sync(0xffffffffu, needl, T - 1);
+                    } else {
+                        if (wait_now && streaming) {
+                            waited(wait_exact<RING_SE * RING_NS / 32>(p, c0, c0 + min(wlen, RING_SE * RING_NS), lane, epoch));
+                            __syncwarp();
+                            if (lane == 0) asm volatile("fence.proxy.async.global;\n" ::: "memory");
+                        }
+                        for (; issued < T && issued < RING_NS; ++issued) issue(issued);
+                    }
+                    auto issue_ready = [&](int cap) {
+                        bool first = true;
+                        while (issued < min(T, cap) && __shfl_sync(0xffffffffu, needl, issued) < tnext) {
+                            if (first && lane == 0) asm volatile("fence.proxy.async.global;\n" ::: "memory");
+                            first = false;
+                            issue(issued++);
+                        }
+                    };
                     int32_t pr_next = -2;
                     if (full == 32) { const int64_t q = c0 + 1024 + 32 * (int64_t)(lane + 1) - 1; pr_next = q < p.N ? __ldg(p.skeys + q) : -2; }
                     for (int ts = 0; ts < T; ++ts) {
                         const int st = ts & (RING_NS - 1);
+                        uint32_t fr[8];
+                        bool scan = false;
+                        if (front) {
+                            if (streaming && issued == ts) {
+                                waited(wait_frontier(p, tnext, __shfl_sync(0xffffffffu, needl, ts), lim, lane, epoch));
+                                __syncwarp();
+                            }
+                            if (streaming) {
+                                issue_ready(ts + RING_NS);
+                                scan = issued < min(T, ts + 1 + RING_NS) && tnext <= lim;
+                                if (scan) frontier_load(p, tnext, lim, lane, epoch, fr);
+                            } else {
+                                while (issued < min(T, ts + RING_NS)) issue(issued++);
+                            }
+                        }
                         long long w0 = 0;
                         if (p.dbg) w0 = clock64();
                         if (!mbar_wait(bars + st, (phase >> st) & 1u)) { ok = false; break; }
@@ -426,7 +553,26 @@
                         __syncwarp();
                         long long w2 = 0;
                         if (p.dbg) { w2 = clock64(); c_cons += w2 - w1; }
-                        if (ts + RING_NS < T) issue(ts + RING_NS);
+                        if (front) {
+                            if (scan) {
+                                const uint32_t pre = frontier_count(fr, tnext, lim, epoch);
+                                if (pre) {
+                                    tnext += pre;
+                                    asm volatile("fence.acq_rel.gpu;\n" ::: "memory");
+                                    __syncwarp();
+                                }
+                            }
+                            if (streaming) issue_ready(ts + 1 + RING_NS);
+                            else while (issued < min(T, ts + 1 + RING_NS)) issue(issued++);
+                        } else if (ts + RING_NS < T) {
+                            if (wait_now && streaming) {
+                                const int64_t a = c0 + RING_SE * (int64_t)(ts + RING_NS);
+                                waited(wait_exact<RING_SE / 32>(p, a, min(a + RING_SE, wend), lane, epoch));
+                                __syncwarp();
+                                if (lane == 0) asm volatile("fence.proxy.async.global;\n" ::: "memory");
+                            }
+                            issue(ts + RING_NS);
+                        }
                         if (p.dbg) c_issue += clock64() - w2;
                     }
                     run_len += wlen;
@@ -482,16 +628,16 @@
 template <bool ADA>
 __global__ void __launch_bounds__(256, 2) fm_bwd_runs_kernel(const __grid_constant__ CUtensorMap gmap, BwdParams p, int warps_per_block, int warp_f,
                                                              int accs_n, int ring_comps) {
-    runs_body<false, 64, 4, false, ADA>(gmap, p, warps_per_block, warp_f, accs_n, ring_comps, blockIdx.x, gridDim.x, 0);
+    runs_body<false, 64, 4, false, ADA>(gmap, p, warps_per_block, warp_f, accs_n, ring_comps, blockIdx.x, gridDim.x, 0, 0u);
 }
 
 constexpr int LONG_SE = 128, LONG_NS = 4;
 template <bool ADA>
 __global__ void __launch_bounds__(256, 2) fm_bwd_runs_list_kernel(const __grid_constant__ CUtensorMap gmap_s, const __grid_constant__ CUtensorMap gmap_l,
                                                                   BwdParams p, int wps, int warp_f_s, int wpl, int warp_f_l, int accs_n,
-                                                                  int ring_comps, unsigned nlong, int segb_off) {
-    if (blockIdx.x < nlong) runs_body<true, LONG_SE, LONG_NS, true, ADA>(gmap_l, p, wpl, warp_f_l, accs_n, ring_comps, blockIdx.x, nlong, segb_off);
-    else runs_body<true, 64, 4, false, ADA>(gmap_s, p, wps, warp_f_s, accs_n, ring_comps, blockIdx.x - nlong, gridDim.x - nlong, segb_off);
+                                                                  int ring_comps, unsigned nlong, int segb_off, uint32_t epoch) {
+    if (blockIdx.x < nlong) runs_body<true, LONG_SE, LONG_NS, true, ADA>(gmap_l, p, wpl, warp_f_l, accs_n, ring_comps, blockIdx.x, nlong, segb_off, epoch);
+    else runs_body<true, 64, 4, false, ADA>(gmap_s, p, wps, warp_f_s, accs_n, ring_comps, blockIdx.x - nlong, gridDim.x - nlong, segb_off, epoch);
 }
 
 static int ilog2_ceil(int x) { int l = 0; while ((1 << l) < x) ++l; return l; }
@@ -540,7 +686,7 @@
 }
 
 template <bool ADA>
-static int launch_runs_t(BwdParams& p, bool two, cudaStream_t stream) {
+static int launch_runs_t(BwdParams& p, bool two, uint32_t epoch, cudaStream_t stream) {
     const int k = p.k;
     const int64_t N = p.N;
     const int nv = k + 1 + (two ? k : 0);
@@ -596,17 +742,17 @@
         at[0].val.programmaticStreamSerializationAllowed = 1;
         cfg.attrs = at; cfg.numAttrs = 1;
         const cudaError_t le = cudaLaunchKernelEx(&cfg, fm_bwd_runs_list_kernel<ADA>, gmap, gmap_l, p, wpb, warp_f, wpl, warp_f_l, accs_n,
-                                                  ring_comps, nlong, (int)(smd / 4));
+                                                  ring_comps, nlong, (int)(smd / 4), epoch);
         if (le != cudaSuccess) { fmb_set_error("fm_bwd_runs_list_kernel (programmatic launch): %s", cudaGetErrorString(le)); return FMB_ERR_CUDA; }
     } else {
         fm_bwd_runs_list_kernel<ADA><<<nlong + nshort, 32 * wpb, smd + segb, stream>>>(gmap, gmap_l, p, wpb, warp_f, wpl, warp_f_l, accs_n,
-                                                                                 ring_comps, nlong, (int)(smd / 4));
+                                                                                 ring_comps, nlong, (int)(smd / 4), epoch);
     }
     FMB_CHECK_LAUNCH("fm_bwd_runs_list_kernel");
     return FMB_OK;
 }
-static int launch_runs(BwdParams& p, bool two, cudaStream_t stream) {
-    return p.mode == 3 ? launch_runs_t<true>(p, two, stream) : launch_runs_t<false>(p, two, stream);
+static int launch_runs(BwdParams& p, bool two, cudaStream_t stream, uint32_t epoch = 0) {
+    return p.mode == 3 ? launch_runs_t<true>(p, two, epoch, stream) : launch_runs_t<false>(p, two, epoch, stream);
 }
 
 struct fmb_runlist_t { int32_t* entries; uint32_t* seg_count; int nseg, seg_cap; };
@@ -698,6 +844,13 @@
 
 static thread_local int g_runs_pdl = 0;
 FMB_API void fmb_runs_list_next_is_dependent(int on) { g_runs_pdl = on; }
+static thread_local struct { const int32_t* perm; const uint32_t* flags; uint32_t epoch; int SB; int* err; } g_runs_stream;
+FMB_API void fmb_runs_list_next_streams(const int32_t* perm, const uint32_t* flags, uint32_t epoch, int SB, int* err) {
+    g_runs_stream.perm = perm; g_runs_stream.flags = flags; g_runs_stream.epoch = epoch; g_runs_stream.SB = SB; g_runs_stream.err = err;
+}
+FMB_API int fmb_is_runs_list_kernel_fn(const void* fn) {
+    return fn == (const void*)fm_bwd_runs_list_kernel<false> || fn == (const void*)fm_bwd_runs_list_kernel<true>;
+}
 
 FMB_API int fmb_fm_backward_runs_list(const int32_t* sorted_keys, int64_t N, float* table, int F, int k, float lr,
                                       int mode, const fmb_ftrl_t* ftrl, const fmb_runlist_t* rl,
@@ -728,8 +881,14 @@
     if (rl) { p.run_list = reinterpret_cast<const int4*>(rl->entries); p.run_segc = rl->seg_count; p.run_nseg = rl->nseg; p.run_cap = rl->seg_cap; }
     p.pdl = rl ? g_runs_pdl : 0;
     g_runs_pdl = 0;
+    const auto st = g_runs_stream;
+    g_runs_stream.flags = nullptr;
+    if (rl && st.flags) {
+        FMB_CHECK_ARG(st.perm && st.err && st.SB > 0, "fmb_fm_backward_runs: bad streaming arguments");
+        p.perm = st.perm; p.sflags = st.flags; p.err = st.err; p.tile_div = (uint32_t)F * (uint32_t)st.SB;
+    }
     p.dbg = g_runs_dbg;
-    return launch_runs(p, false, stream);
+    return launch_runs(p, false, stream, st.epoch);
 }
 
 FMB_API int fmb_fm_backward_runs_ex(const int32_t* sorted_keys, int64_t N, float* table, int F, int k, float lr,
diff --git a/fm_for_online_recommendation_b200/csrc/fm_step.cu b/fm_for_online_recommendation_b200/csrc/fm_step.cu
--- a/fm_for_online_recommendation_b200/csrc/fm_step.cu
+++ b/fm_for_online_recommendation_b200/csrc/fm_step.cu
@@ -34,12 +34,13 @@
     };
     long long* tdbg;
     int dbg;
+    uint32_t* sflags;
 };
 
 template <int CU, bool XV, int MODE>
 __global__ void __launch_bounds__(256, MODE == 2 ? 4 : 8) fm_step_fused_kernel(const int32_t* __restrict__ ids, const float* __restrict__ xv,
                                                             const float* __restrict__ y, const uint32_t* __restrict__ posflag,
-                                                            StepParams p) {
+                                                            StepParams p, uint32_t epoch) {
     extern __shared__ __align__(16) float smem[];
     const int F = p.F, k = p.k, SB = p.SB;
     const int cu = CU ? CU : p.cu;
@@ -147,7 +148,46 @@
     __syncthreads();
     FMB_TS(4);
 
-    const int ns = n_single, nm = n_multi;
+    const int nm = n_multi;
+    if ((p.dbg & 4) && blockIdx.x + 64 >= gridDim.x) {
+        if (threadIdx.x == 0) {
+            unsigned long long t0, t1;
+            asm volatile("mov.u64 %0, %globaltimer;" : "=l"(t0));
+            do { __nanosleep(1000); asm volatile("mov.u64 %0, %globaltimer;" : "=l"(t1)); } while (t1 - t0 < 20000);
+        }
+        __syncthreads();
+    }
+    for (int it = threadIdx.x; it < ((p.dbg & 2) ? 0 : nm * cu); it += blockDim.x) {
+        const int li = fmb_div_by_magic((unsigned)it, p.mcu), q = it - li * cu;
+        const int ef = multi_s[li];
+        const int s = fmb_div_by_magic((unsigned)ef, p.mF);
+        const float x = XV ? x_s[ef] : 1.0f, d = d_s[s];
+        const float4 S4 = *reinterpret_cast<const float4*>(S_s + s * rp + q * 4);
+        const float4 v4 = *reinterpret_cast<const float4*>(rows_s + (size_t)ef * rp + q * 4);
+        const float Sq[4] = {S4.x, S4.y, S4.z, S4.w};
+        const float v[4] = {v4.x, v4.y, v4.z, v4.w};
+        float* g = p.G + (size_t)(q * 4) * p.Npad + (pos_s[ef] & 0x7fffffffu);
+#pragma unroll
+        for (int t = 0; t < 4; ++t) {
+            const int j = q * 4 + t;
+            if (j < k) {
+                const float ej = XV ? __fmul_rn(v[t], x) : v[t];
+                float a = __fsub_rn(__fmul_rn(d, Sq[t]), __fmul_rn(d, ej));
+                if (XV) a = __fmul_rn(a, x);
+                g[(size_t)t * p.Npad] = a;
+            } else if (j == k) {
+                g[(size_t)t * p.Npad] = XV ? __fmul_rn(d, x) : d;
+            }
+        }
+    }
+    if (p.sflags) {
+        __syncthreads();
+        if (threadIdx.x == blockDim.x - 32) {
+            asm volatile("st.release.gpu.global.u32 [%0], %1;\n" ::"l"(p.sflags + blockIdx.x), "r"(epoch) : "memory");
+        }
+    }
+    FMB_TS(5);
+    const int ns = n_single;
     for (int it = threadIdx.x; it < ((p.dbg & 1) ? 0 : ns * cu); it += blockDim.x) {
         const int li = fmb_div_by_magic((unsigned)it, p.mcu), q = it - li * cu;
         const int ef = single_s[li];
@@ -253,30 +293,6 @@
             *reinterpret_cast<float4*>(zrow + p.rowp) = make_float4(nn[0], nn[1], nn[2], nn[3]);
         }
     }
-    FMB_TS(5);
-    for (int it = threadIdx.x; it < ((p.dbg & 2) ? 0 : nm * cu); it += blockDim.x) {
-        const int li = fmb_div_by_magic((unsigned)it, p.mcu), q = it - li * cu;
-        const int ef = multi_s[li];
-        const int s = fmb_div_by_magic((unsigned)ef, p.mF);
-        const float x = XV ? x_s[ef] : 1.0f, d = d_s[s];
-        const float4 S4 = *reinterpret_cast<const float4*>(S_s + s * rp + q * 4);
-        const float4 v4 = *reinterpret_cast<const float4*>(rows_s + (size_t)ef * rp + q * 4);
-        const float Sq[4] = {S4.x, S4.y, S4.z, S4.w};
-        const float v[4] = {v4.x, v4.y, v4.z, v4.w};
-        float* g = p.G + (size_t)(q * 4) * p.Npad + (pos_s[ef] & 0x7fffffffu);
-#pragma unroll
-        for (int t = 0; t < 4; ++t) {
-            const int j = q * 4 + t;
-            if (j < k) {
-                const float ej = XV ? __fmul_rn(v[t], x) : v[t];
-                float a = __fsub_rn(__fmul_rn(d, Sq[t]), __fmul_rn(d, ej));
-                if (XV) a = __fmul_rn(a, x);
-                g[(size_t)t * p.Npad] = a;
-            } else if (j == k) {
-                g[(size_t)t * p.Npad] = XV ? __fmul_rn(d, x) : d;
-            }
-        }
-    }
     FMB_TS(6);
 }
 
@@ -328,10 +344,13 @@
 
 static int g_step_dbg = 0;
 static long long* g_step_tdbg = nullptr;
+static thread_local uint32_t* g_step_sflags = nullptr;
+static thread_local uint32_t g_step_epoch = 0;
+FMB_API void fmb_step_next_signals(uint32_t* flags, uint32_t epoch) { g_step_sflags = flags; g_step_epoch = epoch; }
 FMB_API void fmb_debug_set_step_timestamps(long long* dev) { g_step_tdbg = dev; }
 FMB_API void fmb_debug_set_step_flags(int f) { g_step_dbg = f; }
 
-typedef void (*fused_fn_t)(const int32_t*, const float*, const float*, const uint32_t*, StepParams);
+typedef void (*fused_fn_t)(const int32_t*, const float*, const float*, const uint32_t*, StepParams, uint32_t);
 static fused_fn_t fused_fn(int cu, bool xv, int mode) {
 #define FMB_FUSED_ROW(C, X) {fm_step_fused_kernel<C, X, 0>, fm_step_fused_kernel<C, X, 1>, fm_step_fused_kernel<C, X, 2>, \
                              fm_step_fused_kernel<C, X, 3>}
@@ -369,6 +388,24 @@
 
 struct fmb_ftrl_t { float* zn; float* bias_zn; float beta, l1, l2; };
 struct fmb_adagrad_t { float* sums; float* bias_sum; float* mlp_sums; float eps; };
+
+static size_t step_tile_bytes(int F, int k, int sb) {
+    const int cu = (k + 1 + 3) / 4;
+    return sizeof(float) * ((size_t)sb * F * cu * 4 + (size_t)4 * sb * F + (size_t)sb * k + (size_t)sb * cu * 4 + sb);
+}
+FMB_API int fmb_fm_step_tile_samples(int F, int k) {
+    int SB = 256 >> ilog2_ceil(fmb_round_up(k, 4));
+    if (SB < 4) SB = 4;
+    if (SB > 32) SB = 32;
+    while (SB > 1 && step_tile_bytes(F, k, SB) > 48 * 1024) SB >>= 1;
+    while (SB > 8) SB >>= 1;
+    {
+        static int cap = -1;
+        if (cap < 0) { const char* e = getenv("FMB_STEP_SB"); cap = e ? atoi(e) : 0; }
+        if (cap > 0 && SB > cap) SB = cap;
+    }
+    return step_tile_bytes(F, k, SB) <= 200 * 1024 ? SB : 0;
+}
 
 FMB_API int fmb_fm_step_fused_ex(const int32_t* ids, const float* xv, const float* y, float* table, const float* bias,
                                  const uint32_t* posflag, int B, int F, int k, int loss_kind, float lr, int mode,
@@ -395,25 +432,17 @@
     if (mode == 2) { p.ftrl.zn = ftrl->zn; p.ftrl.bias_zn = ftrl->bias_zn; p.ftrl.beta = ftrl->beta; p.ftrl.l1 = ftrl->l1; p.ftrl.l2 = ftrl->l2; }
     if (mode == 3) { const fmb_adagrad_t* a = reinterpret_cast<const fmb_adagrad_t*>(ftrl); p.ada.sums = a->sums; p.ada.bias_sum = a->bias_sum; p.ada.eps = a->eps; }
     p.tdbg = g_step_tdbg;
-    int SB = 256 >> p.jl_log;
-    if (SB < 4) SB = 4;
-    if (SB > 32) SB = 32;
-    auto bytes = [&](int sb) {
-        return sizeof(float) * ((size_t)sb * F * p.cu * 4 + (size_t)4 * sb * F + (size_t)sb * k + (size_t)sb * p.cu * 4 + sb);
-    };
-    while (SB > 1 && bytes(SB) > 48 * 1024) SB >>= 1;
-    while (SB > 8) SB >>= 1;
-    {
-        static int cap = -1;
-        if (cap < 0) { const char* e = getenv("FMB_STEP_SB"); cap = e ? atoi(e) : 0; }
-        if (cap > 0 && SB > cap) SB = cap;
-    }
-    FMB_CHECK_ARG(bytes(SB) <= 200 * 1024, "fmb_fm_step_fused: F*k too large for one sample tile (F=%d k=%d: %zu bytes > 200 KB)",
-                  F, k, bytes(SB));
+    const int SB = fmb_fm_step_tile_samples(F, k);
+    FMB_CHECK_ARG(SB > 0, "fmb_fm_step_fused: F*k too large for one sample tile (F=%d k=%d: %zu bytes > 200 KB)",
+                  F, k, step_tile_bytes(F, k, 1));
     p.SB = SB;
+    p.sflags = g_step_sflags;
+    const uint32_t epoch = g_step_epoch;
+    g_step_sflags = nullptr; g_step_epoch = 0;
     const fused_fn_t fn = fused_fn(p.cu, xv != nullptr, mode);
-    if (bytes(SB) > 48 * 1024) cudaFuncSetAttribute(fn, cudaFuncAttributeMaxDynamicSharedMemorySize, 200 * 1024);
-    fn<<<(B + SB - 1) / SB, 256, bytes(SB), stream>>>(ids, xv, y, posflag, p);
+    const size_t smem = step_tile_bytes(F, k, SB);
+    if (smem > 48 * 1024) cudaFuncSetAttribute(fn, cudaFuncAttributeMaxDynamicSharedMemorySize, 200 * 1024);
+    fn<<<(B + SB - 1) / SB, 256, smem, stream>>>(ids, xv, y, posflag, p, epoch);
     FMB_CHECK_LAUNCH("fm_step_fused_kernel");
     return FMB_OK;
 }
diff --git a/fm_for_online_recommendation_b200/csrc/session.cu b/fm_for_online_recommendation_b200/csrc/session.cu
--- a/fm_for_online_recommendation_b200/csrc/session.cu
+++ b/fm_for_online_recommendation_b200/csrc/session.cu
@@ -34,6 +34,10 @@
 int fmb_fm_backward_runs(const int32_t*, int64_t, float*, int, int, float, int, void*, size_t, cudaStream_t);
 int fmb_is_fused_kernel_fn(const void*);
 void fmb_runs_list_next_is_dependent(int);
+void fmb_runs_list_next_streams(const int32_t*, const uint32_t*, uint32_t, int, int*);
+int fmb_is_runs_list_kernel_fn(const void*);
+void fmb_step_next_signals(uint32_t*, uint32_t);
+int fmb_fm_step_tile_samples(int, int);
 const void* fmb_finish_kernel_fn(void);
 int fmb_sort_fields_kernel_fns(const void**, int*, int*);
 }
@@ -45,10 +49,11 @@
     float lr;
     cudaGraph_t graph;
     cudaGraphExec_t exec;
-    cudaGraphNode_t n_fused, n_finish, n_sort_cur[2], n_sort_next[2];
+    cudaGraphNode_t n_fused, n_runs, n_finish, n_sort_cur[2], n_sort_next[2];
     int np_sort_cur[2], np_sort_next[2];
     int nlaunch;
     const void *cur_ids, *cur_xv, *cur_y, *cur_sort_ids, *cur_next_ids, *cur_loss;
+    uint32_t cur_epoch;
 };
 
 struct fmb_session {
@@ -112,6 +117,10 @@
     int ftrl_set;
     fmb_adagrad_t ada;
     int ada_set;
+    uint32_t* d_tile_flags;
+    uint32_t epoch;
+    int* h_err;
+    int* d_err;
 };
 
 #define CU(call)                                                                              \
@@ -134,7 +143,8 @@
     if (s->st4) cudaStreamDestroy(s->st4);
     if (s->ev_join4) cudaEventDestroy(s->ev_join4);
     if (s->ev_presort) cudaEventDestroy(s->ev_presort);
-    cudaFree(s->d_sort_ws); cudaFree(s->d_bwd_ws); cudaFree(s->d_field_off);
+    cudaFree(s->d_sort_ws); cudaFree(s->d_bwd_ws); cudaFree(s->d_field_off); cudaFree(s->d_tile_flags);
+    if (s->h_err) cudaFreeHost(s->h_err);
     cudaFreeHost(s->h_ids); cudaFreeHost(s->h_xv); cudaFreeHost(s->h_y); cudaFreeHost(s->h_loss);
     cudaFree(s->d_ids2); cudaFree(s->d_xv2); cudaFree(s->d_y2); cudaFree(s->d_loss2);
     cudaFreeHost(s->h_ids2); cudaFreeHost(s->h_xv2); cudaFreeHost(s->h_y2);
@@ -177,6 +187,10 @@
     if (!(field_off_host && max_batch <= fmb_sort_fields_max_batch())) dm(&s->d_sort_ws2, s->sort_ws_bytes);
     s->d_skeys = s->d_skeys_buf[0]; s->d_perm = s->d_perm_buf[0];
     dm(&s->d_sort_ws, s->sort_ws_bytes); dm(&s->d_bwd_ws, s->bwd_ws_bytes);
+    dm((void**)&s->d_tile_flags, (size_t)max_batch * 4);
+    if (e == cudaSuccess) e = cudaMemset(s->d_tile_flags, 0, (size_t)max_batch * 4);
+    if (e == cudaSuccess) e = cudaHostAlloc((void**)&s->h_err, sizeof(int), cudaHostAllocMapped);
+    if (e == cudaSuccess) { *s->h_err = 0; e = cudaHostGetDevicePointer((void**)&s->d_err, s->h_err, 0); }
     hm((void**)&s->h_ids, N * 4); hm((void**)&s->h_xv, N * 4); hm((void**)&s->h_y, max_batch * 4);
     hm((void**)&s->h_loss, 256);
     dm((void**)&s->d_ids2, N * 4); dm((void**)&s->d_xv2, N * 4); dm((void**)&s->d_y2, max_batch * 4);
@@ -297,7 +311,7 @@
 static int fm_step_launch(fmb_session* s, const int32_t* ids, const float* xv, const float* y, int B, float* table,
                           float* bias, int key_bits, int loss_kind, float lr, int mode, float* loss_dev,
                           const int32_t* next_ids, cudaStream_t main, cudaStream_t side, cudaStream_t side2, int cur,
-                          bool pre, int* nlaunch) {
+                          bool pre, uint32_t epoch, int* nlaunch) {
     const int64_t N = (int64_t)B * s->F;
     int rc;
     *nlaunch = 0;
@@ -315,6 +329,7 @@
     }
     const fmb_ftrl_t* ft = mode == 3 ? (s->ada_set ? reinterpret_cast<const fmb_ftrl_t*>(&s->ada) : nullptr)
                                      : (s->ftrl_set ? &s->ftrl : nullptr);
+    fmb_step_next_signals(s->d_tile_flags, epoch);
     rc = fmb_fm_step_fused_ex(ids, xv, y, table, bias, s->d_posflag_buf[cur], B, s->F, s->k, loss_kind, lr, mode, ft,
                               s->d_delta, s->d_lossv, s->d_bwd_ws, s->bwd_ws_bytes, main);
     if (rc) return rc;
@@ -334,6 +349,7 @@
     if (by_field_sort(s, B)) fmb_runlist_shape(B, s->F, &rl.nseg, &rl.seg_cap);
     else { rl.nseg = 1; rl.seg_cap = (int)(N / 2 + 1); }
     fmb_runs_list_next_is_dependent(s->use_pdl);
+    fmb_runs_list_next_streams(s->d_perm_buf[cur], s->d_tile_flags, epoch, fmb_fm_step_tile_samples(s->F, s->k), s->d_err);
     rc = fmb_fm_backward_runs_list(s->d_skeys_buf[cur], N, table, s->F, s->k, lr, mode, ft, &rl, s->d_bwd_ws, s->bwd_ws_bytes, main);
     if (rc) return rc;
     cudaStreamWaitEvent(main, s->ev_join, 0);
@@ -359,7 +375,7 @@
     int nl = 0;
     CU(cudaStreamBeginCapture(s->st0, cudaStreamCaptureModeThreadLocal));
     const int rc = fm_step_launch(s, ids, xv, y, v->B, table, bias, v->key_bits, v->loss_kind, v->lr, v->mode, s->d_loss,
-                                  next_ids, s->st0, s->st1, s->st2, v->cur, v->pre != 0, &nl);
+                                  next_ids, s->st0, s->st1, s->st2, v->cur, v->pre != 0, s->epoch, &nl);
     cudaError_t e = cudaStreamEndCapture(s->st0, &graph);
     if (rc) { if (graph) cudaGraphDestroy(graph); return rc; }
     if (e != cudaSuccess) { fmb_set_error("graph capture: %s", cudaGetErrorString(e)); return FMB_ERR_CUDA; }
@@ -369,7 +385,7 @@
     const void* sort_fns[8];
     int sort_np[8], sort_ska[8];
     const int nsort = fmb_sort_fields_kernel_fns(sort_fns, sort_np, sort_ska);
-    v->n_fused = v->n_finish = nullptr;
+    v->n_fused = v->n_runs = v->n_finish = nullptr;
     for (int j = 0; j < 2; ++j) v->n_sort_cur[j] = v->n_sort_next[j] = nullptr;
     for (size_t i = 0; i < nn; ++i) {
         cudaGraphNodeType ty;
@@ -378,6 +394,7 @@
         cudaKernelNodeParams kp;
         CU(cudaGraphKernelNodeGetParams(nodes[i], &kp));
         if (fmb_is_fused_kernel_fn(kp.func)) { v->n_fused = nodes[i]; continue; }
+        if (fmb_is_runs_list_kernel_fn(kp.func)) { v->n_runs = nodes[i]; continue; }
         if (kp.func == fmb_finish_kernel_fn()) { v->n_finish = nodes[i]; continue; }
         for (int t = 0; t < nsort; ++t)
             if (kp.func == sort_fns[t]) {
@@ -389,7 +406,7 @@
                 dst[j] = nodes[i]; dnp[j] = sort_np[t];
             }
     }
-    if (!v->n_fused || !v->n_finish || (!v->pre && !v->n_sort_cur[0]) || (v->has_next && !v->n_sort_next[0])) {
+    if (!v->n_fused || !v->n_runs || !v->n_finish || (!v->pre && !v->n_sort_cur[0]) || (v->has_next && !v->n_sort_next[0])) {
         cudaGraphDestroy(graph);
         fmb_set_error("step graph: kernel nodes not found");
         return FMB_ERR_CUDA;
@@ -397,7 +414,7 @@
     cudaGraphExec_t exec = nullptr;
     e = cudaGraphInstantiate(&exec, graph, s->use_prio ? cudaGraphInstantiateFlagUseNodePriority : 0);
     if (e != cudaSuccess) { cudaGraphDestroy(graph); fmb_set_error("graph instantiate: %s", cudaGetErrorString(e)); return FMB_ERR_CUDA; }
-    v->graph = graph; v->exec = exec; v->nlaunch = nl;
+    v->graph = graph; v->exec = exec; v->nlaunch = nl; v->cur_epoch = s->epoch;
     return FMB_OK;
 }
 
@@ -406,6 +423,16 @@
                                      const int32_t* next_ids, float* loss_dev, cudaStream_t stream) {
     FMB_CHECK_ARG(s && ids && y && table && bias, "fmb_session_fm_step: null pointer");
     FMB_CHECK_ARG(B > 0 && B <= s->maxB, "fmb_session_fm_step: B=%d exceeds session max_batch", B);
+    if (*(volatile int*)s->h_err) {
+        *(volatile int*)s->h_err = 0;
+        fmb_set_error("fmb_session_fm_step: the run kernel of an earlier step timed out waiting for the fused kernel's tiles "
+                      "(the rows hit several times in that step were updated from incomplete sums)");
+        return FMB_ERR_CUDA;
+    }
+    if (++s->epoch == 0) {
+        CU(cudaMemsetAsync(s->d_tile_flags, 0, (size_t)s->maxB * 4, stream));
+        s->epoch = 1;
+    }
     int nl = 0;
     const bool pre = s->presort_ids == ids && s->presort_B == B && !s->presort_stale;
     s->presort_stale = 0;
@@ -422,7 +449,7 @@
     int rc = FMB_OK;
     if (!s->use_graph || s->steps_done == 0 || !by_field_sort(s, B)) {
         rc = fm_step_launch(s, ids, xv, y, B, table, bias, key_bits, loss_kind, lr, mode, loss_dev, next_ids, stream,
-                            s->st1, s->st2, cur, pre, &nl);
+                            s->st1, s->st2, cur, pre, s->epoch, &nl);
         if (rc) return rc;
         s->launches += nl;
     } else {
@@ -453,12 +480,20 @@
             s->gvar[slot] = key;
             v = &s->gvar[slot];
         }
-        if (v->cur_ids != ids || v->cur_xv != xv || v->cur_y != y) {
+        const uint32_t ep = s->epoch;
+        if (v->cur_ids != ids || v->cur_xv != xv || v->cur_y != y || v->cur_epoch != ep) {
             const void* repl[16] = {nullptr};
-            repl[0] = &ids; repl[1] = &xv; repl[2] = &y;
-            rc = patch_node(v->exec, v->n_fused, 5, repl);
+            repl[0] = &ids; repl[1] = &xv; repl[2] = &y; repl[5] = &ep;
+            rc = patch_node(v->exec, v->n_fused, 6, repl);
             if (rc) return rc;
             v->cur_ids = ids; v->cur_xv = xv; v->cur_y = y;
+        }
+        if (v->cur_epoch != ep) {
+            const void* repl[16] = {nullptr};
+            repl[11] = &ep;
+            rc = patch_node(v->exec, v->n_runs, 12, repl);
+            if (rc) return rc;
+            v->cur_epoch = ep;
         }
         if (!pre && v->cur_sort_ids != ids) {
             const void* repl[16] = {nullptr};
```

Result: slower. 162.2 million, median of 6 (-20.2%).
